# suhrig/arriba

Hardware: AMD Instinct MI355X
Metric: chimeric reads/s end-to-end (BAM->fusions.tsv), synthetic (higher is better)
Workload: dtype int32

## Files before the change

arriba_amd/csrc/device/agpu_ingest.hip:

```cpp
#include <hip/hip_runtime.h>
#include <algorithm>
#include <cstring>
#include <string>
#include <vector>
#include <rocprim/rocprim.hpp>
#include "agpu_context.hpp"
#include "ingest_core.hpp"
#include "device_utils.hpp"
#include "shard_host.hpp"
#include "crc32_core.hpp"
#include "inflate_fast_core.hpp"

using namespace agpu;
namespace agpu { extern thread_local bool g_inside_ingest_finish; }

namespace {

const int BLOCK = 256;
inline unsigned int grid_for(uint64_t n, int block = BLOCK) { return (unsigned int) ((n + block - 1) / block); }

enum { IC_ACTIVE = 0, IC_MAPPED_READS = 1, IC_MISSING_HI = 2, IC_BROKEN = 3, IC_MALFORMED = 4, IC_CHIMERIC = 5, IC_COLLISION = 6, IC_MISMATCH = 7, IC_UNSORTED = 8, IC_MAX_NAME = 9,
       IC_MAX_READ_LENGTH = 10, IC_STRAND_COUNT = 11, IC_STRAND_MATCHING = 12, IC_RUNS_UNSORTED = 13, IC_QNAME_COMMA = 14, IC_COUNT = 16 };

#define HIP_CHECK(call) do { hipError_t e_ = (call); if (e_ != hipSuccess) { set_last_error(std::string(#call) + ": " + hipGetErrorString(e_)); return AGPU_ERR_DEVICE; } } while (0)
#define ALLOC(buffer, bytes) do { if (!(buffer).allocate(bytes)) { set_last_error("hipMalloc failed (" #buffer ")"); return AGPU_ERR_NO_MEMORY; } } while (0)
#define TRY(call) do { int s_ = (call); if (s_ != AGPU_OK) return s_; } while (0)


__global__ void __launch_bounds__(BLOCK) bgzf_unwrap_kernel(const uint8_t* raw, const agpu_bgzf_block* blocks, uint8_t* stream) {
	const agpu_bgzf_block block = blocks[blockIdx.x];
	const uint8_t* source = raw + block.raw_offset + block.payload_offset;
	uint8_t* target = stream + block.stream_offset;
	const uint32_t size = block.payload_size;
	uint32_t head = (uint32_t) ((4 - ((uintptr_t) target & 3)) & 3);
	if (head > size) head = size;
	if (threadIdx.x < head) target[threadIdx.x] = source[threadIdx.x];
	const uint32_t words = (size - head) / 4;
	for (uint32_t w = threadIdx.x; w < words; w += BLOCK) *(uint32_t*) (target + head + 4 * (size_t) w) = load_u32(source + head + 4 * (size_t) w);
	const uint32_t tail = head + 4 * words;
	if (threadIdx.x < size - tail) target[tail + threadIdx.x] = source[tail + threadIdx.x];
}

template <int LANES> __global__ void __launch_bounds__(LANES) bgzf_inflate_tokens_kernel(const uint8_t* raw, const agpu_bgzf_block* blocks, uint32_t n_blocks, uint8_t* stream, uint8_t* spill,
                                                                                        unsigned long long* notes, uint32_t* note_count, int* status, unsigned int* failures) {
	__shared__ InflateFastTables tables[LANES];
	const uint32_t b = blockIdx.x * LANES + threadIdx.x;
	if (b >= n_blocks) return;
	const agpu_bgzf_block block = blocks[b];
	const bool partial = block.skip != 0 || block.keep != block.isize;
	uint8_t* target = partial ? spill + (b == 0 ? 0 : 65536) : stream + block.stream_offset;
	uint32_t noted = 0;
	const int result = block.isize > 65536 ? (int) INFLATE_OUTPUT_OVERRUN
	                 : inflate_tokens(raw + block.raw_offset + block.payload_offset, block.payload_size, target, block.isize, notes + (size_t) b * INFLATE_MATCH_CAPACITY, INFLATE_MATCH_CAPACITY, noted, tables[threadIdx.x]);
	note_count[b] = noted; status[b] = result;
	if (result != INFLATE_OK && result != INFLATE_RETRY) atomicAdd(failures, 1u);
}

__global__ void __launch_bounds__(BLOCK) bgzf_inflate_resolve_kernel(const agpu_bgzf_block* blocks, uint32_t n_blocks, uint8_t* stream, uint8_t* spill, const unsigned long long* notes, const uint32_t* note_count, const int* status) {
	const uint32_t b = blockIdx.x * (BLOCK / 64) + (threadIdx.x >> 6), lane = threadIdx.x & 63;
	if (b >= n_blocks || status[b] != INFLATE_OK) return;
	const agpu_bgzf_block block = blocks[b];
	const bool partial = block.skip != 0 || block.keep != block.isize;
	uint8_t* target = partial ? spill + (b == 0 ? 0 : 65536) : stream + block.stream_offset;
	const unsigned long long* mine = notes + (size_t) b * INFLATE_MATCH_CAPACITY;
	const uint32_t n = note_count[b];
	for (uint32_t base = 0; base < n; base += 64) {
		const unsigned long long note = base + lane < n ? mine[base + lane] : 0ull;
		const uint32_t position = inflate_note_position(note), length = inflate_note_length(note), distance = inflate_note_distance(note);
		bool pending = base + lane < n;
		while (true) {
			const unsigned long long waiting = __ballot(pending);
			if (waiting == 0) break;
			const uint32_t frontier = (uint32_t) __shfl((int) position, __ffsll((unsigned long long) waiting) - 1);
			if (pending && inflate_match_is_ready(position, length, distance, frontier)) { inflate_copy_match(target, position, length, distance); pending = false; }
			__builtin_amdgcn_fence(__ATOMIC_SEQ_CST, "workgroup");
		}
	}
	if (partial) for (uint32_t k = lane; k < block.keep; k += 64) stream[block.stream_offset + k] = target[block.skip + k];
}

__global__ void __launch_bounds__(64, 3) bgzf_inflate_kernel(const uint8_t* raw, const agpu_bgzf_block* blocks, uint8_t* stream, uint8_t* spill, int* status, int* verdict, unsigned int* failures) {
	__shared__ InflateShared shared;
	if (status != nullptr && status[blockIdx.x] != INFLATE_RETRY) return;
	const agpu_bgzf_block block = blocks[blockIdx.x];
	const bool partial = block.skip != 0 || block.keep != block.isize;
	uint8_t* target = partial ? spill + (blockIdx.x == 0 ? 0 : 65536) : stream + block.stream_offset;
	auto sync = [] () { __syncthreads(); };
	auto broadcast = [] (uint32_t value) { return (uint32_t) __builtin_amdgcn_readfirstlane((int) value); };
	const int result = inflate_block(raw + block.raw_offset + block.payload_offset, block.payload_size, target, block.isize, shared, threadIdx.x, 64u, sync, broadcast);
	if (verdict != nullptr && threadIdx.x == 0) verdict[blockIdx.x] = result;
	if (result != INFLATE_OK) { if (threadIdx.x == 0) atomicAdd(failures, 1u); return; }
	if (partial) {
		__syncthreads();
		for (uint32_t k = threadIdx.x; k < block.keep; k += 64) stream[block.stream_offset + k] = __hip_atomic_load(&target[block.skip + k], __ATOMIC_RELAXED, __HIP_MEMORY_SCOPE_AGENT);
	}
}


__global__ void segment_guess_kernel(const uint8_t* bytes, uint64_t size, uint64_t base, uint64_t segment_begin, uint64_t n_segments, uint32_t n_targets, uint64_t* first, uint64_t* end, uint32_t* count) {
	const uint64_t s = segment_begin + blockIdx.x * (uint64_t) BLOCK + threadIdx.x;
	if (s < n_segments) guess_segment(bytes, size, base, s, n_targets, first, end, count);
}

__global__ void segment_check_kernel(const uint64_t* first, const uint64_t* end, uint64_t segment_begin, uint64_t n_segments, uint8_t* mismatch, uint32_t* mismatches) {
	__shared__ uint32_t block_sum;
	uint32_t mine = 0;
	for (uint64_t s = segment_begin + blockIdx.x * (uint64_t) BLOCK + threadIdx.x; s < n_segments; s += gridDim.x * (uint64_t) BLOCK) {
		const bool bad = s > 0 && first[s] != end[s - 1];
		mismatch[s] = bad;
		mine += bad;
	}
	block_tally(mine, mismatches, &block_sum);
}

__global__ void segment_repair_kernel(const uint8_t* bytes, uint64_t size, uint64_t base, uint64_t segment_begin, uint64_t n_segments, const uint8_t* mismatch, const uint64_t* previous_end, uint64_t* first, uint64_t* end, uint32_t* count) {
	const uint64_t s = segment_begin + blockIdx.x * (uint64_t) BLOCK + threadIdx.x;
	if (s < n_segments) repair_segment_run(bytes, size, base, n_segments, s, mismatch, previous_end, first, end, count);
}

__global__ void segment_emit_kernel(const uint8_t* bytes, uint64_t size, uint64_t base, uint64_t segment_begin, uint64_t n_segments, const uint64_t* first, const uint32_t* record_base, uint64_t* record_offset) {
	const uint64_t s = segment_begin + blockIdx.x * (uint64_t) BLOCK + threadIdx.x;
	if (s >= n_segments) return;
	const uint64_t begin = base + s * SEGMENT_BYTES, segment_end = (begin + SEGMENT_BYTES < size) ? begin + SEGMENT_BYTES : size;
	uint32_t n = 0;
	walk_segment(bytes, size, first[s], segment_end, n, record_offset + record_base[s]);
}


const uint32_t PARSE_WINDOW = 16384;
__global__ void __launch_bounds__(BLOCK) record_parse_kernel(IngestStream in, GenomeView genome, uint64_t seed, uint64_t record_begin, uint64_t* keys, uint8_t* bits, int32_t* hit_index, uint32_t* counters) {
	__shared__ uint32_t sums[4];
	__shared__ __attribute__((aligned(16))) uint8_t staged[BLOCK / 64][PARSE_WINDOW + 64];
	const uint32_t wave = threadIdx.x / 64, lane = threadIdx.x % 64;
	uint8_t* window = staged[wave];
	uint32_t active = 0, mapped = 0, missing = 0, broken = 0;
	for (uint64_t base = record_begin + ((uint64_t) blockIdx.x * (BLOCK / 64) + wave) * 64; base < in.n_records; base += (uint64_t) gridDim.x * BLOCK) {
		const uint64_t r = base + lane;
		const uint64_t piece_begin = in.record_offset[base] & ~15ull, piece_end = base + 64 < in.n_records ? in.record_offset[base + 64] : in.size;
		const bool in_lds = piece_end > piece_begin && piece_end - piece_begin <= PARSE_WINDOW;
		if (in_lds) {
			for (uint64_t at = piece_begin + 16 * lane; at < piece_end; at += 16 * 64) *(uint4*) (window + (at - piece_begin)) = *(const uint4*) (in.bytes + at);
			__builtin_amdgcn_fence(__ATOMIC_RELEASE, "workgroup"); __builtin_amdgcn_wave_barrier(); __builtin_amdgcn_fence(__ATOMIC_ACQUIRE, "workgroup");
		}
		if (r < in.n_records) {
			const uint64_t offset = in.record_offset[r];
			const uint8_t* p = in.bytes + offset;
			uint32_t block_size = load_u32(p);
			if (in_lds && offset + 4 + (uint64_t) block_size <= piece_end && offset + 36 <= piece_end) { p = window + (offset - piece_begin); block_size = load_u32(p); }
			uint64_t key = ~0ull;
			uint8_t status = RECORD_SKIPPED;
			int32_t hit = HIT_INDEX_UNKNOWN;
			if (!record_sizes_ok(p + 4, block_size)) { status = RECORD_BROKEN; ++broken; }
			else {
				const Rec record = load_record_at(in, p);
				if (!((record.flag & BAMF_UNMAP) || ((record.flag & BAMF_PAIRED) && (record.flag & BAMF_MUNMAP)))) {
					const AuxTags tags = scan_aux(record.aux, record.end);
					if (!tags.has_hi && (record.flag & BAMF_SECONDARY)) { status = RECORD_MISSING_HI; ++missing; }
					else if (record.contig < 0) { status = RECORD_BROKEN; ++broken; }
					else {
						status = RECORD_ACTIVE | (tags.has_sa ? RECORD_HAS_SA : 0);
						key = name_key(record, tags.has_hi ? tags.hi : 1, seed);
						hit = hit_index_to_keep(tags);
						++active;
						if (!(record.flag & BAMF_SUPPLEMENTARY) && (genome.contig_bits[record.contig] & CBIT_INTERESTING)) ++mapped;
					}
				}
			}
			keys[r] = key;
			bits[r] = status;
			hit_index[r] = hit;
		}
		__builtin_amdgcn_fence(__ATOMIC_RELEASE, "workgroup"); __builtin_amdgcn_wave_barrier();
	}
	block_tally(active, &counters[IC_ACTIVE], &sums[0]);
	block_tally(mapped, &counters[IC_MAPPED_READS], &sums[1]);
	block_tally(missing, &counters[IC_MISSING_HI], &sums[2]);
	block_tally(broken, &counters[IC_BROKEN], &sums[3]);
}

__global__ void group_head_kernel(const uint64_t* sorted_keys, uint64_t n_active, uint8_t* head) {
	const uint64_t p = blockIdx.x * (uint64_t) BLOCK + threadIdx.x;
	if (p < n_active) head[p] = p == 0 || sorted_keys[p] != sorted_keys[p - 1];
}
__global__ void group_first_flag_kernel(const uint32_t* sorted_records, const uint32_t* group_start, uint32_t n_groups, uint8_t* first_flags) {
	const uint32_t g = blockIdx.x * BLOCK + threadIdx.x;
	if (g < n_groups) first_flags[sorted_records[group_start[g]]] = 1;
}
__global__ void group_rank_kernel(const uint32_t* sorted_records, const uint32_t* group_start, uint32_t n_groups, uint64_t n_active, const uint32_t* stream_rank, uint32_t* group_first, uint32_t* group_begin, uint32_t* group_count) {
	const uint32_t g = blockIdx.x * BLOCK + threadIdx.x;
	if (g >= n_groups) return;
	const uint32_t begin = group_start[g], first = sorted_records[begin], t = stream_rank[first];
	group_first[t] = first; group_begin[t] = begin; group_count[t] = (uint32_t) ((g + 1 < n_groups ? (uint64_t) group_start[g + 1] : n_active) - begin);
}
__global__ void group_names_kernel(IngestStream in, const uint32_t* sorted_records, const uint32_t* group_begin, const uint32_t* group_count, uint32_t first_group, uint32_t n_groups, uint32_t* counters) {
	const uint32_t t = first_group + blockIdx.x * BLOCK + threadIdx.x;
	if (t >= n_groups || group_count[t] < 2) return;
	const uint32_t* records = sorted_records + group_begin[t];
	const Rec a = load_record(in, records[0]);
	const int64_t hit_a = hit_index_of(in, records[0], a);
	for (uint32_t k = 1; k < group_count[t]; ++k) {
		const Rec b = load_record(in, records[k]);
		if (!same_name(a, hit_a, b, hit_index_of(in, records[k], b))) { atomicOr(&counters[IC_COLLISION], 1u); return; }
	}
}


__global__ void window_carry_kernel(uint32_t* record_base, uint64_t segment_begin, uint64_t segment_end, const uint32_t* records_before) {
	const uint64_t s = segment_begin + blockIdx.x * (uint64_t) BLOCK + threadIdx.x;
	if (s <= segment_end) record_base[s] += *records_before;
}
__global__ void window_summary_kernel(const uint32_t* record_base, const uint64_t* end, uint64_t segment_end, uint32_t* records_before, uint32_t* words) {
	*records_before = record_base[segment_end];
	words[1] = record_base[segment_end];
	const uint64_t last_end = end[segment_end - 1];
	words[4] = (uint32_t) last_end; words[5] = (uint32_t) (last_end >> 32);
}
struct RecordIsActive { __host__ __device__ bool operator()(uint8_t bits) const { return (bits & RECORD_STATUS_MASK) == RECORD_ACTIVE; } };
__global__ void run_head_kernel(const uint64_t* keys, const uint32_t* active_records, uint64_t begin, uint64_t end, uint8_t* head) {
	const uint64_t i = begin + blockIdx.x * (uint64_t) BLOCK + threadIdx.x;
	if (i < end) head[i] = i == 0 || keys[active_records[i]] != keys[active_records[i - 1]];
}
__global__ void run_close_kernel(const uint32_t* active_records, const uint32_t* run_begin, uint32_t first_group, uint32_t n_groups, uint32_t n_runs, uint64_t active_total, uint32_t* group_first, uint32_t* group_count) {
	const uint32_t g = first_group + blockIdx.x * BLOCK + threadIdx.x;
	if (g >= n_groups) return;
	const uint32_t begin = run_begin[g];
	group_first[g] = active_records[begin];
	group_count[g] = (uint32_t) ((g + 1 < n_runs ? (uint64_t) run_begin[g + 1] : active_total) - begin);
}
__global__ void run_key_kernel(const uint64_t* keys, const uint32_t* group_first, uint32_t n_groups, uint64_t* out) {
	const uint32_t g = blockIdx.x * BLOCK + threadIdx.x;
	if (g < n_groups) out[g] = keys[group_first[g]];
}
__global__ void run_repeat_kernel(const uint64_t* sorted_keys, uint32_t n_groups, uint32_t* repeats) {
	__shared__ uint32_t block_sum;
	uint32_t mine = 0;
	for (uint64_t g = blockIdx.x * (uint64_t) BLOCK + threadIdx.x; g < n_groups; g += gridDim.x * (uint64_t) BLOCK) mine += g > 0 && sorted_keys[g] == sorted_keys[g - 1];
	block_tally(mine, repeats, &block_sum);
}

struct ViralCounter {
	unsigned long long* counts;
	__device__ void operator()(uint32_t contig) { atomicAdd(&counts[contig], 1ull); }
};

#ifndef AGPU_REPLAY_WAVES
#define AGPU_REPLAY_WAVES 0
#endif
#ifndef AGPU_PACK_WAVES
#define AGPU_PACK_WAVES 0
#endif
#if AGPU_REPLAY_WAVES > 0
#define AGPU_REPLAY_OCCUPANCY __attribute__((amdgpu_waves_per_eu(AGPU_REPLAY_WAVES, AGPU_REPLAY_WAVES)))
#else
#define AGPU_REPLAY_OCCUPANCY
#endif
#if AGPU_PACK_WAVES > 0
#define AGPU_PACK_OCCUPANCY __attribute__((amdgpu_waves_per_eu(AGPU_PACK_WAVES, AGPU_PACK_WAVES)))
#else
#define AGPU_PACK_OCCUPANCY
#endif
template <bool RUNS> __global__ void __launch_bounds__(BLOCK) AGPU_REPLAY_OCCUPANCY group_replay_kernel(IngestContext ctx, const uint32_t* sorted_records, const uint32_t* group_begin, const uint32_t* group_count, uint32_t first_group, uint32_t n_groups,
                                                             FragmentPlan* plain, TandemPlan* itd, uint8_t* valid, FragmentSizes* sizes, unsigned long long* viral_counts, uint32_t* qname_differs, uint32_t* counters) {
	__shared__ uint32_t sums[2];
	GroupTally tally; tally.malformed = 0; tally.chimeric = 0; tally.collision = 0;
	const uint32_t g = first_group + blockIdx.x * BLOCK + threadIdx.x;
	if (g < n_groups) {
		const uint32_t begin = group_begin[g];
		const uint32_t n_records = group_count[g];
		const Rec representative = load_record(ctx.stream, sorted_records[begin]);
		const int64_t hit = hit_index_of(ctx.stream, sorted_records[begin], representative);
		const uint32_t length = qname_length(representative);
		if (RUNS) {
			if (find_byte(representative.name, length, ',') < length) atomicOr(&counters[IC_QNAME_COMMA], 1u);
			if (g == 0) qname_differs[0] = 0;
			else {
				const uint32_t record_before = sorted_records[group_begin[g - 1]];
				const Rec run_before = load_record(ctx.stream, record_before);
				const uint32_t length_before = qname_length(run_before), shorter = length < length_before ? length : length_before, different = first_difference(run_before.name, representative.name, shorter);
				qname_differs[g] = length != length_before || different < shorter;
				bool unsorted;
				if (different < shorter) unsorted = run_before.name[different] > representative.name[different];
				else unsorted = compare_names(fragment_name(run_before, hit_index_of(ctx.stream, record_before, run_before), false, length_before), fragment_name(representative, hit, false, length)) >= 0;
				if (unsorted) atomicOr(&counters[IC_RUNS_UNSORTED], 1u);
			}
		}
		FragmentPlan plain_plan; TandemPlan itd_plan;
		ViralCounter viral = { viral_counts };
		replay_group(ctx, sorted_records + begin, n_records, plain_plan, itd_plan, tally, viral, RUNS ? &representative : nullptr, length, hit);
		if (tally.collision) atomicOr(&counters[IC_COLLISION], 1u);
		Fragment3 fragment;
		AGPU_NOUNROLL for (uint32_t entry = 0; entry < 2; ++entry) {
			const FragmentPlan& plan = entry ? itd_plan.plan : plain_plan;
			bool ok = false;
			if (plan.count > 0) {
				ok = normalize_plan(ctx.stream, plan, entry ? &itd_plan.tandem : nullptr, fragment);
				if (!ok) tally.malformed++;
			}
			valid[2 * (size_t) g + entry] = ok;
			FragmentSizes mine; mine.cigar_words = 0; mine.sequence_bytes = 0; mine.name_length = 0;
			if (ok) { if (entry) itd[g] = itd_plan; else plain[g] = plain_plan; fragment_sizes(fragment, representative, hit, entry, mine, length); }
			sizes[2 * (size_t) g + entry] = mine;
		}
	}
	block_tally(tally.malformed, &counters[IC_MALFORMED], &sums[0]);
	block_tally(tally.chimeric, &counters[IC_CHIMERIC], &sums[1]);
}


__device__ FragmentName name_of(const IngestStream& in, const uint32_t* group_first, uint32_t ref, Rec& storage) {
	storage = load_record(in, group_first[ref >> 1]);
	return fragment_name(storage, hit_index_of(in, group_first[ref >> 1], storage), ref & 1);
}

__global__ void name_order_check_kernel(IngestStream in, const uint32_t* group_first, const uint32_t* order, uint64_t n, uint32_t* counters) {
	__shared__ uint32_t block_max;
	if (threadIdx.x == 0) block_max = 0;
	__syncthreads();
	const uint64_t i = blockIdx.x * (uint64_t) BLOCK + threadIdx.x;
	if (i < n) {
		Rec storage_a, storage_b;
		const FragmentName mine = name_of(in, group_first, order[i], storage_a);
		atomicMax(&block_max, name_length(mine));
		if (i > 0) {
			const FragmentName before = name_of(in, group_first, order[i - 1], storage_b);
			if (compare_names(before, mine) >= 0) atomicOr(&counters[IC_UNSORTED], 1u);
		}
	}
	__syncthreads();
	if (threadIdx.x == 0 && block_max) atomicMax(&counters[IC_MAX_NAME], block_max);
}

__global__ void run_itd_order_kernel(IngestStream in, const uint32_t* group_first, const uint8_t* valid, uint32_t first_group, uint32_t n_groups, uint32_t* counters) {
	const uint32_t g = first_group + blockIdx.x * BLOCK + threadIdx.x;
	if (g >= n_groups || g == 0 || !valid[2 * (size_t) (g - 1) + 1]) return;
	Rec storage_a, storage_b;
	const FragmentName mine = name_of(in, group_first, 2 * g, storage_b);
	const FragmentName before = name_of(in, group_first, 2 * (g - 1) + 1, storage_a);
	if (compare_names(before, mine) >= 0) atomicOr(&counters[IC_RUNS_UNSORTED], 1u);
}

__global__ void name_chunk_kernel(IngestStream in, const uint32_t* group_first, const uint32_t* order, uint64_t n, uint32_t chunk, uint64_t* keys) {
	const uint64_t i = blockIdx.x * (uint64_t) BLOCK + threadIdx.x;
	if (i >= n) return;
	Rec storage;
	keys[i] = name_chunk(name_of(in, group_first, order[i], storage), chunk);
}


__global__ void fragment_layout_kernel(IngestStream in, const uint32_t* group_first, const uint32_t* order, uint64_t n, const FragmentSizes* sizes, const uint32_t* qname_run ,
                                       uint32_t* cigar_words, uint32_t* sequence_bytes, uint32_t* name_lengths, uint32_t* new_group) {
	const uint64_t i = blockIdx.x * (uint64_t) BLOCK + threadIdx.x;
	if (i > n) return;
	if (i == n) { cigar_words[i] = 0; sequence_bytes[i] = 0; name_lengths[i] = 0; return; }
	const uint32_t ref = order[i];
	const FragmentSizes mine = sizes[ref];
	cigar_words[i] = mine.cigar_words; sequence_bytes[i] = mine.sequence_bytes; name_lengths[i] = mine.name_length;
	uint32_t differs = 0;
	if (i > 0 && qname_run != nullptr) differs = qname_run[ref >> 1] != qname_run[order[i - 1] >> 1];
	else if (i > 0) {
		const Rec a = load_record(in, group_first[ref >> 1]), b = load_record(in, group_first[order[i - 1] >> 1]);
		const uint32_t length = qname_length(a);
		differs = length != qname_length(b);
		for (uint32_t k = 0; k < length && !differs; ++k) differs = a.name[k] != b.name[k];
	}
	new_group[i] = differs;
}

__global__ void __launch_bounds__(BLOCK) AGPU_PACK_OCCUPANCY fragment_pack_kernel(IngestStream in, const uint32_t* group_first, const uint32_t* order, uint64_t n, const FragmentPlan* plain, const TandemPlan* itd,
                                                              const uint64_t* cigar_base, const uint64_t* sequence_base, const uint64_t* name_base, const uint32_t* group_id, PackTarget out, uint32_t* counters) {
	__shared__ uint32_t block_max;
	if (threadIdx.x == 0) block_max = 0;
	__syncthreads();
	const uint64_t i = blockIdx.x * (uint64_t) BLOCK + threadIdx.x;
	if (i == n) out.name_offset[n] = name_base[n];
	if (i < n) {
		const uint32_t ref = order[i], g = ref >> 1;
		const bool is_itd = ref & 1;
		Fragment3 f;
		normalize_plan(in, is_itd ? itd[g].plan : plain[g], is_itd ? &itd[g].tandem : nullptr, f);
		Rec storage;
		const FragmentName name = name_of(in, group_first, ref, storage);
		atomicMax(&block_max, write_fragment(in, f, name, i, cigar_base[i], sequence_base[i], name_base[i], group_id[i], out));
	}
	__syncthreads();
	if (threadIdx.x == 0 && block_max) atomicMax(&counters[IC_MAX_READ_LENGTH], block_max);
}

template <bool INFLATED> __global__ void __launch_bounds__(256) bgzf_crc_kernel(const uint8_t* raw, const agpu_bgzf_block* blocks, uint32_t n_blocks, const Crc32Tables* tables, unsigned int* mismatches) {
	__shared__ uint32_t slice[4][256];
	__shared__ uint32_t join[2][4][256];
	__shared__ uint32_t staged[4][CRC32_WAVE_LANES * (CRC32_ROUND_WORDS + 1)];
	for (uint32_t k = threadIdx.x; k < 4 * 256; k += 256) ((uint32_t*) slice)[k] = ((const uint32_t*) tables->slice)[k];
	for (uint32_t k = threadIdx.x; k < 2 * 4 * 256; k += 256) ((uint32_t*) join)[k] = ((const uint32_t*) tables->join)[k];
	const uint32_t wave = threadIdx.x / CRC32_WAVE_LANES, lane = threadIdx.x % CRC32_WAVE_LANES, b = blockIdx.x * 4 + wave;
	agpu_bgzf_block block;
	block.crc32 = 0; block.payload_size = 0; block.raw_offset = 0; block.payload_offset = 0;
	if (b < n_blocks) block = blocks[b];
	if (INFLATED) { block.raw_offset = block.stream_offset; block.payload_offset = 0; block.payload_size = block.isize; }
	const bool checked = b < n_blocks && block.crc32 != 0 && block.payload_size <= CRC32_VIRTUAL;
	const uint8_t* payload = raw + block.raw_offset + block.payload_offset;
	const uint32_t n = block.payload_size;
	uint32_t* mine = staged[wave];
	uint32_t c = 0;
	const bool by_chunks = checked && n >= 4;
	const uint32_t first_word = by_chunks ? (CRC32_VIRTUAL - n) / 4 : CRC32_VIRTUAL / 4;
	for (uint32_t round = 0; round < CRC32_WAVE_CHUNK / 4 / CRC32_ROUND_WORDS; ++round) {
		__syncthreads();
		for (uint32_t item = lane; item < CRC32_WAVE_LANES * CRC32_ROUND_WORDS; item += CRC32_WAVE_LANES) {
			const uint32_t chunk = item / CRC32_ROUND_WORDS, j = item % CRC32_ROUND_WORDS, w = chunk * (CRC32_WAVE_CHUNK / 4) + round * CRC32_ROUND_WORDS + j;
			mine[chunk * (CRC32_ROUND_WORDS + 1) + j] = w >= first_word ? crc32_virtual_word(payload, n, w) : 0u;
		}
		__syncthreads();
		for (uint32_t j = 0; j < CRC32_ROUND_WORDS; ++j) c = crc32_raw_step(slice, c, mine[lane * (CRC32_ROUND_WORDS + 1) + j]);
	}
	__syncthreads();
	mine[lane] = c;
	__syncthreads();
	if (lane % 8 == 0) { for (uint32_t i = 1; i < 8; ++i) c = crc32_apply(join[0], c) ^ mine[lane + i]; }
	__syncthreads();
	if (lane % 8 == 0) mine[lane] = c;
	__syncthreads();
	if (lane == 0 && checked) {
		for (uint32_t g = 1; g < 8; ++g) c = crc32_apply(join[1], c) ^ mine[8 * g];
		c ^= 0xFFFFFFFFu;
		if (n < 4) c = crc32_of_sliced(slice, payload, n);
		if (c != block.crc32) atomicAdd(mismatches, 1u);
	}
}

__global__ void shard_rebase_kernel(uint32_t* out, const uint32_t* in, uint64_t n, uint32_t base, const uint8_t* n_aln, uint32_t slot) {
	const uint64_t i = (uint64_t) blockIdx.x * blockDim.x + threadIdx.x;
	if (i < n) out[i] = in[i] + ((slot >= 3 || slot < n_aln[i]) ? base : 0u);
}
__global__ void shard_rebase_names_kernel(uint64_t* out, const uint64_t* in, uint64_t n, uint64_t base) {
	const uint64_t i = (uint64_t) blockIdx.x * blockDim.x + threadIdx.x;
	if (i < n) out[i] = in[i] + base;
}
__global__ void shard_add_coverage_kernel(uint32_t* windows, uint8_t* starts, uint8_t* ends, const uint32_t* part_windows, const uint8_t* part_starts, const uint8_t* part_ends, uint64_t n) {
	const uint64_t i = (uint64_t) blockIdx.x * blockDim.x + threadIdx.x;
	if (i < n) { windows[i] += part_windows[i]; starts[i] |= part_starts[i]; ends[i] |= part_ends[i]; }
}
__global__ void shard_add_counts_kernel(unsigned long long* counts, const unsigned long long* part, uint32_t n) {
	const uint32_t i = blockIdx.x * blockDim.x + threadIdx.x;
	if (i < n) counts[i] += part[i];
}

__global__ void packed_name_length_kernel(const uint64_t* name_offset, uint64_t n, uint32_t* longest) {
	const uint64_t i = blockIdx.x * (uint64_t) BLOCK + threadIdx.x;
	if (i < n) atomicMax(longest, (uint32_t) (name_offset[i + 1] - name_offset[i]));
}
__global__ void packed_name_chunk_kernel(const char* names, const uint64_t* name_offset, const uint32_t* order, uint64_t n, uint32_t chunk, uint64_t* keys) {
	const uint64_t i = blockIdx.x * (uint64_t) BLOCK + threadIdx.x;
	if (i >= n) return;
	const uint32_t row = order[i]; const uint64_t begin = name_offset[row]; const uint32_t length = (uint32_t) (name_offset[row + 1] - begin);
	uint64_t key = 0;
	for (uint32_t k = 0; k < 8; ++k) { const uint32_t at = 8 * chunk + k; key = key << 8 | (at < length ? (uint8_t) names[begin + at] : 0u); }
	keys[i] = key;
}
__global__ void packed_name_neighbours_kernel(const char* names, const uint64_t* name_offset, const uint32_t* order, uint64_t n, uint32_t* new_group, uint32_t* equal_names) {
	const uint64_t i = blockIdx.x * (uint64_t) BLOCK + threadIdx.x;
	if (i >= n) return;
	if (i == 0) { new_group[0] = 0; return; }
	const uint32_t a = order[i - 1], b = order[i]; const uint64_t begin_a = name_offset[a], begin_b = name_offset[b]; const uint32_t length_a = (uint32_t) (name_offset[a + 1] - begin_a), length_b = (uint32_t) (name_offset[b + 1] - begin_b);
	bool same = length_a == length_b;
	for (uint32_t k = 0; same && k < length_a; ++k) same = names[begin_a + k] == names[begin_b + k];
	if (same) atomicAdd(equal_names, 1u);
	uint32_t qname_a = length_a, qname_b = length_b;
	while (qname_a > 0 && names[begin_a + qname_a - 1] != ',') --qname_a;
	while (qname_b > 0 && names[begin_b + qname_b - 1] != ',') --qname_b;
	bool same_qname = qname_a == qname_b;
	for (uint32_t k = 0; same_qname && k < qname_a; ++k) same_qname = names[begin_a + k] == names[begin_b + k];
	new_group[i] = same_qname ? 0u : 1u;
}
__global__ void qname_run_flag_kernel(IngestStream in, uint64_t n_records, uint8_t* flags) {
	const uint64_t r = blockIdx.x * (uint64_t) BLOCK + threadIdx.x;
	if (r < n_records) flags[r] = starts_qname_run(in, (uint32_t) r) ? 1 : 0;
}
__global__ void qname_key_kernel(IngestStream in, const uint32_t* run_starts, uint64_t n_runs, uint64_t* keys) {
	const uint64_t k = blockIdx.x * (uint64_t) BLOCK + threadIdx.x;
	if (k < n_runs) qname_key128(load_record(in, run_starts[k]), keys[2 * k], keys[2 * k + 1]);
}
__global__ void qname_low_kernel(const uint64_t* keys, uint64_t n, uint64_t* low) { const uint64_t k = blockIdx.x * (uint64_t) BLOCK + threadIdx.x; if (k < n) low[k] = keys[2 * k]; }
__global__ void qname_equal_kernel(const uint64_t* low_sorted, const uint32_t* index_sorted, const uint64_t* keys, uint64_t n, uint32_t* equal) {
	const uint64_t k = blockIdx.x * (uint64_t) BLOCK + threadIdx.x;
	if (k > 0 && k < n && low_sorted[k] == low_sorted[k - 1] && keys[2 * (uint64_t) index_sorted[k] + 1] == keys[2 * (uint64_t) index_sorted[k - 1] + 1]) atomicAdd(equal, 1u);
}
__global__ void iota_kernel(uint32_t* out, uint64_t n) { const uint64_t i = blockIdx.x * (uint64_t) BLOCK + threadIdx.x; if (i < n) out[i] = (uint32_t) i; }

__global__ void coverage_from_differences_kernel(const uint32_t* summed, const uint64_t* window_offset, uint32_t n_contigs, uint64_t n, uint32_t* counts, uint16_t* out) {
	const uint64_t i = blockIdx.x * (uint64_t) BLOCK + threadIdx.x;
	if (i >= n) return;
	uint32_t low = 0, high = n_contigs;
	while (high - low > 1) { const uint32_t middle = (low + high) / 2; if (window_offset[middle] <= i) low = middle; else high = middle; }
	const uint32_t count = summed[i + low];
	counts[i] = count;
	out[i] = count > 65535u ? (uint16_t) 65535 : (uint16_t) count;
}
__global__ void coverage_clamp_kernel(const uint32_t* windows, uint64_t n, uint16_t* out) {
	const uint64_t i = blockIdx.x * (uint64_t) BLOCK + threadIdx.x;
	if (i < n) out[i] = windows[i] > 65535u ? (uint16_t) 65535 : (uint16_t) windows[i];
}


__global__ void gather_sizes_kernel(BatchView b, const uint64_t* name_offset, const uint32_t* ids, uint64_t n, uint32_t* cigar_words, uint32_t* sequence_bytes, uint32_t* name_lengths) {
	const uint64_t k = blockIdx.x * (uint64_t) BLOCK + threadIdx.x;
	if (k > n) return;
	if (k == n) { cigar_words[k] = 0; sequence_bytes[k] = 0; name_lengths[k] = 0; return; }
	row_sizes(b, name_offset, ids ? ids[k] : k, cigar_words[k], sequence_bytes[k], name_lengths[k]);
}

__global__ void gather_copy_kernel(BatchView b, const uint8_t* pristine_fbits, const uint8_t* const* pristine_abits, const uint64_t* name_offset, const char* names, const uint32_t* ids, uint64_t n,
                                   const uint64_t* cigar_base, const uint64_t* sequence_base, const uint64_t* name_base, PackTarget out) {
	const uint64_t k = blockIdx.x * (uint64_t) BLOCK + threadIdx.x;
	if (k == n) { if (out.name_offset) out.name_offset[n] = name_base[n]; else out.row_name_offset[n] = (uint32_t) name_base[n]; }
	if (k >= n) return;
	copy_row(b, pristine_fbits, pristine_abits, name_offset, names, ids ? ids[k] : k, k, cigar_base[k], sequence_base[k], name_base[k], out);
}


__global__ void strandedness_flag_kernel(BatchView b, AnnotationView ann, uint64_t first, uint64_t count, uint8_t* flags) {
	const uint64_t k = blockIdx.x * (uint64_t) BLOCK + threadIdx.x;
	if (k >= count) return;
	flags[k] = strandedness_vote(b, ann, first + k);
}

__global__ void strandedness_take_kernel(const uint8_t* flags, uint64_t count, uint32_t wanted, uint32_t* counters) {
	if (blockIdx.x != 0 || threadIdx.x != 0) return;
	uint32_t seen = counters[IC_STRAND_COUNT], matching = counters[IC_STRAND_MATCHING];
	for (uint64_t k = 0; k < count && seen < wanted; ++k)
		if (flags[k]) { ++seen; if (flags[k] & 2) ++matching; }
	counters[IC_STRAND_COUNT] = seen; counters[IC_STRAND_MATCHING] = matching;
}


int grow_stream(agpu_ctx* ctx, uint64_t needed) {
	needed += 64;
	if (needed <= ctx->ingest_stream.capacity) { ctx->ingest_stream.bytes = needed; return AGPU_OK; }
	DeviceBuffer larger;
	const uint64_t doubled = ctx->ingest_stream.capacity * 2;
	if (!larger.allocate(std::max<uint64_t>(needed + (needed >> 3), std::max<uint64_t>(doubled, 64u << 20)))) { set_last_error("hipMalloc failed (BAM stream)"); return AGPU_ERR_NO_MEMORY; }
	if (ctx->piece_stream) { HIP_CHECK(hipStreamSynchronize(ctx->piece_stream)); HIP_CHECK(hipStreamSynchronize(ctx->piece_stream2)); }
	if (ctx->ingest_stream_size > 0) HIP_CHECK(hipMemcpyAsync(larger.ptr, ctx->ingest_stream.ptr, ctx->ingest_stream_size, hipMemcpyDeviceToDevice, ctx->stream));
	HIP_CHECK(hipStreamSynchronize(ctx->stream));
	if (ctx->ingest_progress.work) HIP_CHECK(hipStreamSynchronize(ctx->ingest_progress.work));
	ctx->ingest_stream.swap(larger);
	return AGPU_OK;
}

int wait_for_previous_push(agpu_ctx* ctx) {
	const uint32_t behind = ctx->ingest_host_buffers - 1;
	if (ctx->ingest_pushes >= behind) HIP_CHECK(hipEventSynchronize(ctx->piece_copied[(ctx->ingest_pushes - behind) % AGPU_PIECE_SLOTS]));
	return AGPU_OK;
}

template <class Key> int sort_pairs(agpu_ctx* ctx, DeviceBuffer& scratch, Key* keys_in, Key* keys_out, uint32_t* values_in, uint32_t* values_out, uint64_t n, unsigned int end_bit, const char* label, bool counting_values) {
	size_t bytes = 0;
	hipStream_t s = ctx->stream;
	if (counting_values) HIP_CHECK(rocprim::radix_sort_pairs(nullptr, bytes, keys_in, keys_out, rocprim::counting_iterator<uint32_t>(0), values_out, n, 0, end_bit, s));
	else HIP_CHECK(rocprim::radix_sort_pairs(nullptr, bytes, keys_in, keys_out, values_in, values_out, n, 0, end_bit, s));
	if (bytes > scratch.capacity) ALLOC(scratch, bytes);
	KernelTimer timer(ctx, label, n * (uint64_t) (sizeof(Key) + 4) * 2);
	if (counting_values) HIP_CHECK(rocprim::radix_sort_pairs(scratch.ptr, bytes, keys_in, keys_out, rocprim::counting_iterator<uint32_t>(0), values_out, n, 0, end_bit, s));
	else HIP_CHECK(rocprim::radix_sort_pairs(scratch.ptr, bytes, keys_in, keys_out, values_in, values_out, n, 0, end_bit, s));
	return AGPU_OK;
}

int select_flagged(agpu_ctx* ctx, DeviceBuffer& scratch, const uint8_t* flags, uint32_t* out, uint32_t* device_count, uint64_t n) {
	size_t bytes = 0;
	HIP_CHECK(rocprim::select(nullptr, bytes, rocprim::counting_iterator<uint32_t>(0), flags, out, device_count, n, ctx->stream));
	if (bytes > scratch.capacity) ALLOC(scratch, bytes);
	HIP_CHECK(rocprim::select(scratch.ptr, bytes, rocprim::counting_iterator<uint32_t>(0), flags, out, device_count, n, ctx->stream));
	return AGPU_OK;
}

int exclusive_sum_u64(agpu_ctx* ctx, DeviceBuffer& scratch, const uint32_t* in, uint64_t* out, uint64_t n) {
	size_t bytes = 0;
	HIP_CHECK(rocprim::exclusive_scan(nullptr, bytes, in, out, (uint64_t) 0, n, rocprim::plus<uint64_t>(), ctx->stream));
	if (bytes > scratch.capacity) ALLOC(scratch, bytes);
	HIP_CHECK(rocprim::exclusive_scan(scratch.ptr, bytes, in, out, (uint64_t) 0, n, rocprim::plus<uint64_t>(), ctx->stream));
	return AGPU_OK;
}


const unsigned int INGEST_WINDOW_RING = 16, INGEST_WINDOW_WORDS = 8;
uint64_t g_window_bytes = 512u << 20;
uint64_t g_window_margin = 1u << 20;

int grow_keeping(agpu_ctx* ctx, DeviceBuffer& buffer, size_t needed, size_t used, size_t estimate) {
	if (needed == 0) needed = 16;
	if (buffer.ptr != nullptr && needed <= buffer.capacity) { if (needed > buffer.bytes) buffer.bytes = needed; return AGPU_OK; }
	DeviceBuffer larger;
	if (!larger.allocate(std::max(needed + needed / 2, estimate)) && !larger.allocate(needed)) { set_last_error("hipMalloc failed (tables of the ingest)"); return AGPU_ERR_NO_MEMORY; }
	hipStream_t s = ctx->ingest_progress.work;
	if (used > 0 && buffer.ptr != nullptr) HIP_CHECK(hipMemcpyAsync(larger.ptr, buffer.ptr, std::min(used, buffer.capacity), hipMemcpyDeviceToDevice, s));
	HIP_CHECK(hipStreamSynchronize(s));
	buffer.swap(larger);
	return AGPU_OK;
}

IngestStream window_stream(agpu_ctx* ctx, uint64_t size, uint64_t n_records) {
	IngestStream in;
	in.bytes = ctx->ingest_stream.as<uint8_t>(); in.size = size; in.record_offset = ctx->scratch("ingest.record_offset").as<uint64_t>(); in.n_records = n_records;
	in.n_targets = ctx->ingest_n_targets; in.tid_to_contig = ctx->ingest_tid_to_contig.as<uint32_t>();
	in.hit_index = ctx->scratch("ingest.hit_index").as<int32_t>();
	return in;
}

IngestContext replay_context(agpu_ctx* ctx, const IngestStream& in) {
	IngestContext context;
	context.stream = in; context.annotation = ctx->annotation; context.annotation.n_dummy = 0; context.genome = ctx->genome;
	context.coverage.n_contigs = ctx->genome.n_contigs; context.coverage.window_offset = ctx->coverage_window_offset.as<uint64_t>(); context.coverage.windows = ctx->coverage_windows32.as<uint32_t>();
	context.coverage.fragment_starts = ctx->coverage_fragment_starts.as<uint8_t>(); context.coverage.fragment_ends = ctx->coverage_fragment_ends.as<uint8_t>();
	if (getenv("ARRIBA_INGEST_SKIP_COVERAGE") != nullptr) context.coverage.windows = nullptr;
	context.record_bits = ctx->scratch("ingest.record_bits").as<uint8_t>(); context.max_itd_length = ctx->ingest_max_itd_length; context.external_duplicate_marking = ctx->ingest_external_duplicate_marking;
	return context;
}

int window_step(agpu_ctx* ctx, IngestWindow& w) {
	IngestProgress& p = ctx->ingest_progress;
	hipStream_t s = p.work;
	uint32_t* words = ctx->scratch("ingest.window_words").as<uint32_t>() + (size_t) w.slot * INGEST_WINDOW_WORDS;
	uint32_t* device_counters = ctx->scratch("ingest.counters").as<uint32_t>();
	DeviceBuffer& rocprim_scratch = ctx->scratch("ingest.window_rocprim");
	const uint64_t base = ctx->ingest_first_record;
	const uint8_t* bytes = ctx->ingest_stream.as<uint8_t>();
	const uint64_t n = w.segment_end - w.segment_begin;
	const size_t estimated_records = (size_t) (p.size_hint / 128 + 4096);
	size_t temporary = 0;
	switch (w.enqueued + 1) {
	case 1: {
		HIP_CHECK(hipMemsetAsync(words, 0, INGEST_WINDOW_WORDS * 4, s));
		if (n == 0) break;
		DeviceBuffer& first = ctx->scratch("ingest.segment_first"); DeviceBuffer& end = ctx->scratch("ingest.segment_end"); DeviceBuffer& end_before = ctx->scratch("ingest.segment_end_before");
		DeviceBuffer& count = ctx->scratch("ingest.segment_count"); DeviceBuffer& record_base = ctx->scratch("ingest.segment_base"); DeviceBuffer& mismatch = ctx->scratch("ingest.segment_mismatch");
		const size_t segments = (size_t) w.segment_end + 1, done = (size_t) w.segment_begin + 1, estimate = (size_t) (p.size_hint / SEGMENT_BYTES + 16);
		TRY(grow_keeping(ctx, first, segments * 8, done * 8, estimate * 8)); TRY(grow_keeping(ctx, end, segments * 8, done * 8, estimate * 8)); TRY(grow_keeping(ctx, end_before, segments * 8, 0, estimate * 8));
		TRY(grow_keeping(ctx, count, segments * 4, done * 4, estimate * 4)); TRY(grow_keeping(ctx, record_base, segments * 4, done * 4, estimate * 4)); TRY(grow_keeping(ctx, mismatch, segments, done, estimate));
		{ KernelTimer timer(ctx, "segment_guess_kernel", n * SEGMENT_BYTES, s);
		  segment_guess_kernel<<<grid_for(n), BLOCK, 0, s>>>(bytes, w.avail, base, w.segment_begin, w.segment_end, ctx->ingest_n_targets, first.as<uint64_t>(), end.as<uint64_t>(), count.as<uint32_t>()); }
		for (int pass = 0; pass < 3; ++pass) {
			segment_check_kernel<<<tally_grid(n, BLOCK), BLOCK, 0, s>>>(first.as<uint64_t>(), end.as<uint64_t>(), w.segment_begin, w.segment_end, mismatch.as<uint8_t>(), words + 6);
			const uint64_t from = w.segment_begin > 0 ? w.segment_begin - 1 : 0;
			HIP_CHECK(hipMemcpyAsync(end_before.as<uint64_t>() + from, end.as<uint64_t>() + from, (w.segment_end - from) * 8, hipMemcpyDeviceToDevice, s));
			segment_repair_kernel<<<grid_for(n), BLOCK, 0, s>>>(bytes, w.avail, base, w.segment_begin, w.segment_end, mismatch.as<uint8_t>(), end_before.as<uint64_t>(), first.as<uint64_t>(), end.as<uint64_t>(), count.as<uint32_t>());
		}
		segment_check_kernel<<<tally_grid(n, BLOCK), BLOCK, 0, s>>>(first.as<uint64_t>(), end.as<uint64_t>(), w.segment_begin, w.segment_end, mismatch.as<uint8_t>(), words + 0);
		HIP_CHECK(hipMemsetAsync(count.as<uint32_t>() + w.segment_end, 0, 4, s));
		HIP_CHECK(rocprim::exclusive_scan(nullptr, temporary, count.as<uint32_t>() + w.segment_begin, record_base.as<uint32_t>() + w.segment_begin, 0u, n + 1, rocprim::plus<uint32_t>(), s));
		if (temporary > rocprim_scratch.capacity) ALLOC(rocprim_scratch, temporary);
		HIP_CHECK(rocprim::exclusive_scan(rocprim_scratch.ptr, temporary, count.as<uint32_t>() + w.segment_begin, record_base.as<uint32_t>() + w.segment_begin, 0u, n + 1, rocprim::plus<uint32_t>(), s));
		uint32_t* records_before = ctx->scratch("ingest.window_state").as<uint32_t>();
		window_carry_kernel<<<grid_for(n + 1), BLOCK, 0, s>>>(record_base.as<uint32_t>(), w.segment_begin, w.segment_end, records_before);
		window_summary_kernel<<<1, 1, 0, s>>>(record_base.as<uint32_t>(), end.as<uint64_t>(), w.segment_end, records_before, words);
		break; }
	case 2: {
		const uint64_t records = w.record_end - w.record_begin;
		w.active_begin = p.active;
		if (records == 0) break;
		DeviceBuffer& record_offset = ctx->scratch("ingest.record_offset"); DeviceBuffer& keys = ctx->scratch("ingest.keys"); DeviceBuffer& record_bits = ctx->scratch("ingest.record_bits"); DeviceBuffer& active_records = ctx->scratch("ingest.sorted_records");
		TRY(grow_keeping(ctx, record_offset, w.record_end * 8, w.record_begin * 8, estimated_records * 8)); TRY(grow_keeping(ctx, keys, w.record_end * 8, w.record_begin * 8, estimated_records * 8));
		TRY(grow_keeping(ctx, ctx->scratch("ingest.hit_index"), w.record_end * 4, w.record_begin * 4, estimated_records * 4));
		TRY(grow_keeping(ctx, record_bits, w.record_end, w.record_begin, estimated_records)); TRY(grow_keeping(ctx, active_records, (w.active_begin + records) * 4, w.active_begin * 4, estimated_records * 4));
		{ KernelTimer timer(ctx, "segment_emit_kernel", records * 8, s);
		  segment_emit_kernel<<<grid_for(n), BLOCK, 0, s>>>(bytes, w.avail, base, w.segment_begin, w.segment_end, ctx->scratch("ingest.segment_first").as<uint64_t>(), ctx->scratch("ingest.segment_base").as<uint32_t>(), record_offset.as<uint64_t>()); }
		const IngestStream in = window_stream(ctx, w.avail, w.record_end);
		{ KernelTimer timer(ctx, "record_parse_kernel", records * (8 + 64 + 9), s);
		  record_parse_kernel<<<tally_grid(records, BLOCK) * 8, BLOCK, 0, s>>>(in, ctx->genome, 0, w.record_begin, keys.as<uint64_t>(), record_bits.as<uint8_t>(), ctx->scratch("ingest.hit_index").as<int32_t>(), device_counters); }
		auto flags = rocprim::make_transform_iterator(record_bits.as<uint8_t>() + w.record_begin, RecordIsActive());
		HIP_CHECK(rocprim::select(nullptr, temporary, rocprim::counting_iterator<uint32_t>((uint32_t) w.record_begin), flags, active_records.as<uint32_t>() + w.active_begin, words + 2, records, s));
		if (temporary > rocprim_scratch.capacity) ALLOC(rocprim_scratch, temporary);
		HIP_CHECK(rocprim::select(rocprim_scratch.ptr, temporary, rocprim::counting_iterator<uint32_t>((uint32_t) w.record_begin), flags, active_records.as<uint32_t>() + w.active_begin, words + 2, records, s));
		break; }
	case 3: {
		const uint64_t active = w.active_end - w.active_begin;
		w.head_begin = p.heads;
		if (active == 0) break;
		DeviceBuffer& head = ctx->scratch("ingest.head"); DeviceBuffer& run_begin = ctx->scratch("ingest.group_begin");
		TRY(grow_keeping(ctx, head, w.active_end, 0, estimated_records)); TRY(grow_keeping(ctx, run_begin, (w.head_begin + active + 1) * 4, w.head_begin * 4, estimated_records * 2));
		{ KernelTimer timer(ctx, "run_head_kernel", active * (8 + 4 + 1), s);
		  run_head_kernel<<<grid_for(active), BLOCK, 0, s>>>(ctx->scratch("ingest.keys").as<uint64_t>(), ctx->scratch("ingest.sorted_records").as<uint32_t>(), w.active_begin, w.active_end, head.as<uint8_t>()); }
		HIP_CHECK(rocprim::select(nullptr, temporary, rocprim::counting_iterator<uint32_t>((uint32_t) w.active_begin), head.as<uint8_t>() + w.active_begin, run_begin.as<uint32_t>() + w.head_begin, words + 3, active, s));
		if (temporary > rocprim_scratch.capacity) ALLOC(rocprim_scratch, temporary);
		HIP_CHECK(rocprim::select(rocprim_scratch.ptr, temporary, rocprim::counting_iterator<uint32_t>((uint32_t) w.active_begin), head.as<uint8_t>() + w.active_begin, run_begin.as<uint32_t>() + w.head_begin, words + 3, active, s));
		break; }
	case 4: {
// ... 1161 lines not shown
```

arriba_amd/csrc/device/ingest_core.hpp:

```cpp
#ifndef AGPU_INGEST_CORE_HPP
#define AGPU_INGEST_CORE_HPP 1

#include "annotate_core.hpp"
#include "event_core.hpp"

namespace agpu {


AGPU_HD uint32_t load_u32(const uint8_t* p) { uint32_t v; __builtin_memcpy(&v, p, 4); return v; }
AGPU_HD uint64_t load_u64(const uint8_t* p) { uint64_t v; __builtin_memcpy(&v, p, 8); return v; }
AGPU_HD uint32_t first_zero_byte(uint64_t v) { const uint64_t z = (v - 0x0101010101010101ull) & ~v & 0x8080808080808080ull; return z ? (uint32_t) __builtin_ctzll(z) >> 3 : 8u; }
AGPU_HD uint64_t low_bytes(uint32_t n) { return n >= 8 ? ~0ull : (1ull << (8 * n)) - 1; }
AGPU_HD uint32_t find_byte(const uint8_t* p, uint32_t n, uint8_t byte) {
	const uint64_t pattern = 0x0101010101010101ull * byte;
	uint32_t i = 0;
	for (; i + 8 <= n; i += 8) { const uint32_t z = first_zero_byte(load_u64(p + i) ^ pattern); if (z < 8) return i + z; }
	if (i == n) return n;
	if (n >= 8) {
		const uint32_t z = first_zero_byte((load_u64(p + n - 8) ^ pattern) | low_bytes(i - (n - 8)));
		return z < 8 ? n - 8 + z : n;
	}
	for (; i < n; ++i) if (p[i] == byte) return i;
	return n;
}
AGPU_HD uint32_t first_difference(const uint8_t* a, const uint8_t* b, uint32_t n) {
	uint32_t i = 0;
	for (; i + 8 <= n; i += 8) { const uint64_t x = load_u64(a + i) ^ load_u64(b + i); if (x) return i + ((uint32_t) __builtin_ctzll(x) >> 3); }
	if (i == n) return n;
	if (n >= 8) {
		const uint64_t x = (load_u64(a + n - 8) ^ load_u64(b + n - 8)) & ~low_bytes(i - (n - 8));
		return x ? n - 8 + ((uint32_t) __builtin_ctzll(x) >> 3) : n;
	}
	for (; i < n; ++i) if (a[i] != b[i]) return i;
	return n;
}
AGPU_HD uint16_t load_u16(const uint8_t* p) { uint16_t v; __builtin_memcpy(&v, p, 2); return v; }

enum : uint16_t { BAMF_PAIRED = 1, BAMF_PROPER_PAIR = 2, BAMF_UNMAP = 4, BAMF_MUNMAP = 8, BAMF_REVERSE = 16, BAMF_READ1 = 64, BAMF_SECONDARY = 256, BAMF_DUP = 1024, BAMF_SUPPLEMENTARY = 2048 };

AGPU_HD bool op_consumes_query(uint32_t op) { return (0x3C1A7u >> (op << 1)) & 1; }
AGPU_HD bool op_consumes_reference(uint32_t op) { return (0x3C1A7u >> (op << 1)) & 2; }

struct IngestStream {
	const uint8_t* bytes;
	uint64_t size;
	const uint64_t* record_offset;
	uint64_t n_records;
	uint32_t n_targets;
	const uint32_t* tid_to_contig;
	const int32_t* hit_index;
};
const int32_t HIT_INDEX_UNKNOWN = -0x7FFFFFFF - 1;

struct Rec {
	const uint8_t* cigar_bytes; const uint8_t* seq_bytes; const uint8_t* name; const uint8_t* aux; const uint8_t* end;
	int32_t contig, pos, l_seq;
	uint32_t n_cigar, l_read_name;
	uint16_t flag;
	AGPU_HD uint32_t cigar(uint32_t i) const { return load_u32(cigar_bytes + 4 * (size_t) i); }
	AGPU_HD uint32_t op(uint32_t i) const { return cigar(i) & 15; }
	AGPU_HD uint32_t len(uint32_t i) const { return cigar(i) >> 4; }
	AGPU_HD uint32_t code(int32_t i) const { return (seq_bytes[i >> 1] >> ((~i & 1) << 2)) & 15; }
	AGPU_HD bool forward() const { return !(flag & BAMF_REVERSE); }
	AGPU_HD bool paired() const { return flag & BAMF_PAIRED; }
	AGPU_HD int32_t qlen(uint32_t n) const { int32_t l = 0; for (uint32_t i = 0; i < n; ++i) if (op_consumes_query(op(i))) l += (int32_t) len(i); return l; }
	AGPU_HD int32_t rlen(uint32_t n) const { int32_t l = 0; for (uint32_t i = 0; i < n; ++i) if (op_consumes_reference(op(i))) l += (int32_t) len(i); return l; }
	AGPU_HD int32_t endpos() const { int32_t l = (!(flag & BAMF_UNMAP) && n_cigar > 0) ? rlen(n_cigar) : 1; return pos + (l == 0 ? 1 : l); }
};

AGPU_HD bool record_sizes_ok(const uint8_t* block, uint32_t block_size) {
	if (block_size < 32) return false;
	const uint32_t l_read_name = block[8], n_cigar = load_u16(block + 12);
	const int32_t l_seq = (int32_t) load_u32(block + 16);
	if (l_seq < 0 || l_read_name == 0) return false;
	const uint64_t fixed = 32ull + l_read_name + 4ull * n_cigar + ((uint64_t) l_seq + 1) / 2 + (uint64_t) l_seq;
	return fixed <= block_size;
}

AGPU_HD Rec load_record_at(const IngestStream& in, const uint8_t* p) {
	const uint64_t word0 = load_u64(p), word1 = load_u64(p + 8), word2 = load_u64(p + 16);
	const uint32_t block_size = (uint32_t) word0;
	p += 4;
	Rec rec;
	const int32_t tid = (int32_t) (word0 >> 32);
	rec.contig = (tid >= 0 && (uint32_t) tid < in.n_targets) ? (int32_t) in.tid_to_contig[tid] : -1;
	rec.pos = (int32_t) (uint32_t) word1;
	rec.l_read_name = (uint32_t) (word1 >> 32) & 0xFFu;
	rec.n_cigar = (uint32_t) word2 & 0xFFFFu;
	rec.flag = (uint16_t) (word2 >> 16);
	rec.l_seq = (int32_t) (word2 >> 32);
	rec.name = p + 32;
	rec.cigar_bytes = rec.name + rec.l_read_name;
	rec.seq_bytes = rec.cigar_bytes + 4 * (size_t) rec.n_cigar;
	rec.aux = rec.seq_bytes + ((size_t) rec.l_seq + 1) / 2 + (size_t) rec.l_seq;
	rec.end = p + block_size;
	return rec;
}
AGPU_HD Rec load_record(const IngestStream& in, uint32_t r) { return load_record_at(in, in.bytes + in.record_offset[r]); }


const uint32_t SEGMENT_BYTES = 8192;
const uint64_t SEARCH_LIMIT = 4u << 20;
const uint64_t OFFSET_NONE = ~0ull, OFFSET_BROKEN = ~0ull - 1;

AGPU_HD bool plausible_record(const uint8_t* bytes, uint64_t size, uint64_t o, uint32_t n_targets) {
	if (o + 36 > size) return false;
	const uint32_t block_size = load_u32(bytes + o);
	if (block_size < 32 || block_size > (1u << 28) || o + 4 + (uint64_t) block_size > size) return false;
	const uint8_t* p = bytes + o + 4;
	const int32_t tid = (int32_t) load_u32(p), pos = (int32_t) load_u32(p + 4), next_tid = (int32_t) load_u32(p + 20), next_pos = (int32_t) load_u32(p + 24);
	if (tid < -1 || tid >= (int32_t) n_targets || next_tid < -1 || next_tid >= (int32_t) n_targets || pos < -1 || next_pos < -1) return false;
	if (!record_sizes_ok(p, block_size)) return false;
	const uint32_t l_read_name = p[8];
	return p[32 + l_read_name - 1] == 0;
}

AGPU_HD uint64_t walk_segment(const uint8_t* bytes, uint64_t size, uint64_t start, uint64_t segment_end, uint32_t& count, uint64_t* offsets) {
	uint64_t o = start;
	count = 0;
	while (o < segment_end) {
		if (o + 4 > size) return OFFSET_BROKEN;
		const uint32_t block_size = load_u32(bytes + o);
		if (block_size < 32 || o + 4 + (uint64_t) block_size > size) return OFFSET_BROKEN;
		if (offsets != nullptr) offsets[count] = o;
		++count;
		o += 4 + (uint64_t) block_size;
	}
	return o;
}

AGPU_HD void guess_segment(const uint8_t* bytes, uint64_t size, uint64_t base, uint64_t s, uint32_t n_targets, uint64_t* first, uint64_t* end, uint32_t* count) {
	const uint64_t begin = base + s * SEGMENT_BYTES, segment_end = (begin + SEGMENT_BYTES < size) ? begin + SEGMENT_BYTES : size;
	uint64_t start = OFFSET_NONE;
	if (s == 0) start = base;
	else {
		const uint64_t limit = (begin + SEARCH_LIMIT < size) ? begin + SEARCH_LIMIT : size;
		for (uint64_t o = begin; o < limit; ++o) {
			if (!plausible_record(bytes, size, o, n_targets)) continue;
			const uint64_t next = o + 4 + (uint64_t) load_u32(bytes + o);
			if (next == size || plausible_record(bytes, size, next, n_targets)) { start = o; break; }
		}
	}
	first[s] = start;
	uint32_t n = 0;
	end[s] = (start == OFFSET_NONE) ? OFFSET_NONE : walk_segment(bytes, size, start, segment_end, n, nullptr);
	count[s] = n;
}

AGPU_HD void repair_segment_run(const uint8_t* bytes, uint64_t size, uint64_t base, uint64_t n_segments, uint64_t s, const uint8_t* mismatch, const uint64_t* previous_end, uint64_t* first, uint64_t* end, uint32_t* count) {
	if (!mismatch[s] || mismatch[s - 1]) return;
	uint64_t start = previous_end[s - 1];
	for (uint64_t t = s; t < n_segments && (t == s || mismatch[t]); ++t) {
		const uint64_t begin = base + t * SEGMENT_BYTES, segment_end = (begin + SEGMENT_BYTES < size) ? begin + SEGMENT_BYTES : size;
		first[t] = start;
		uint32_t n = 0;
		end[t] = (start >= OFFSET_BROKEN) ? start : walk_segment(bytes, size, start, segment_end, n, nullptr);
		count[t] = n;
		start = end[t];
	}
}

struct AuxTags { bool has_hi, has_sa; int64_t hi; };
AGPU_HD AuxTags scan_aux(const uint8_t* s, const uint8_t* end) {
	AuxTags tags; tags.has_hi = false; tags.has_sa = false; tags.hi = 0;
	while (s + 3 <= end) {
		const uint8_t* value = s + 2;
		size_t size;
		switch (*value) {
			case 'A': case 'c': case 'C': size = 2; break;
			case 's': case 'S': size = 3; break;
			case 'i': case 'I': case 'f': size = 5; break;
			case 'd': size = 9; break;
			case 'Z': case 'H': { const uint8_t* p = value + 1; while (p < end && *p) ++p; if (p >= end) return tags; size = (size_t) (p - value) + 1; break; }
			case 'B': {
				if (value + 6 > end) return tags;
				const size_t element = (value[1] == 'c' || value[1] == 'C') ? 1 : (value[1] == 's' || value[1] == 'S') ? 2 : 4;
				size = 6 + element * (size_t) load_u32(value + 2);
				break;
			}
			default: return tags;
		}
		if (value + size > end) return tags;
		if (s[0] == 'H' && s[1] == 'I' && !tags.has_hi) {
			tags.has_hi = true;
			switch (*value) {
				case 'c': tags.hi = (int8_t) value[1]; break;
				case 'C': tags.hi = value[1]; break;
				case 's': tags.hi = (int16_t) load_u16(value + 1); break;
				case 'S': tags.hi = load_u16(value + 1); break;
				case 'i': tags.hi = (int32_t) load_u32(value + 1); break;
				case 'I': tags.hi = load_u32(value + 1); break;
				default: tags.hi = 0; break;
			}
		}
		if (s[0] == 'S' && s[1] == 'A') tags.has_sa = true;
		if (tags.has_hi && tags.has_sa) return tags;
		s = value + size;
	}
	return tags;
}

AGPU_HD int32_t hit_index_to_keep(const AuxTags& tags) { const int64_t hi = tags.has_hi ? tags.hi : 1; return (hi > HIT_INDEX_UNKNOWN && hi <= 0x7FFFFFFF) ? (int32_t) hi : HIT_INDEX_UNKNOWN; }
AGPU_HD int64_t hit_index_of(const IngestStream& in, uint32_t record, const Rec& rec) {
	if (in.hit_index != nullptr) { const int32_t kept = in.hit_index[record]; if (kept != HIT_INDEX_UNKNOWN) return kept; }
	const AuxTags tags = scan_aux(rec.aux, rec.end);
	return tags.has_hi ? tags.hi : 1;
}

enum : uint8_t { RECORD_SKIPPED = 0, RECORD_ACTIVE = 1, RECORD_MISSING_HI = 2, RECORD_BROKEN = 3, RECORD_STATUS_MASK = 3, RECORD_HAS_SA = 4 };

AGPU_HD uint32_t qname_length(const Rec& r) { return find_byte(r.name, r.l_read_name, 0); }

AGPU_HD bool starts_qname_run(const IngestStream& in, uint32_t record) {
	if (record == 0) return true;
	const Rec a = load_record(in, record - 1), b = load_record(in, record);
	const uint32_t length = qname_length(b);
	if (qname_length(a) != length) return true;
	for (uint32_t i = 0; i < length; ++i) if (a.name[i] != b.name[i]) return true;
	return false;
}
AGPU_HD void qname_key128(const Rec& r, uint64_t& low, uint64_t& high) {
	uint64_t h = 1469598103934665603ull, g = 0x9AE16A3B2F90404Full;
	for (uint32_t i = 0; i < r.l_read_name && r.name[i]; ++i) { h = (h ^ r.name[i]) * 1099511628211ull; g = (g ^ (r.name[i] + 0x9Eu)) * 0x100000001B3ull; g ^= g >> 29; }
	h ^= h >> 33; h *= 0xFF51AFD7ED558CCDull; h ^= h >> 33; h *= 0xC4CEB9FE1A85EC53ull; h ^= h >> 33;
	g ^= g >> 31; g *= 0x7FB5D329728EA185ull; g ^= g >> 27; g *= 0x81DADEF4BC2DD44Dull; g ^= g >> 33;
	low = h; high = g;
}

AGPU_HD uint64_t name_key(const Rec& r, int64_t hit_index, uint64_t seed) {
	uint64_t h = 1469598103934665603ull ^ seed;
	for (uint32_t i = 0; i < r.l_read_name && r.name[i]; ++i) h = (h ^ r.name[i]) * 1099511628211ull;
	h ^= (uint64_t) hit_index * 0x9E3779B97F4A7C15ull;
	h ^= h >> 33; h *= 0xFF51AFD7ED558CCDull; h ^= h >> 33; h *= 0xC4CEB9FE1A85EC53ull; h ^= h >> 33;
	return h == ~0ull ? ~0ull - 1 : h;
}
AGPU_HD bool same_name(const Rec& a, uint32_t length_a , int64_t hi_a, const Rec& b, int64_t hi_b) {
	if (hi_a != hi_b) return false;
	if (length_a != qname_length(b)) return false;
	return first_difference(a.name, b.name, length_a) == length_a;
}
AGPU_HD bool same_name(const Rec& a, int64_t hi_a, const Rec& b, int64_t hi_b) { return same_name(a, qname_length(a), hi_a, b, hi_b); }


enum : uint8_t { CLIP_NONE = 0, CLIP_START = 1, CLIP_END = 2, PLAN_TANDEM = 3 };
const uint32_t NO_RECORD = 0xFFFFFFFFu;

struct PlanEntry { uint32_t record; uint16_t cigar_index; uint8_t clip; uint8_t supplementary; };
struct TandemAlignment { int32_t start, end; uint32_t cigar[3]; uint32_t record; uint8_t n_cigar, strand, first_in_pair, supplementary; };
struct FragmentPlan {
	PlanEntry entry[3];
	uint8_t count;
	uint8_t single_end, duplicate, reserved;
};
struct TandemPlan { FragmentPlan plan; TandemAlignment tandem; };

AGPU_HD void plan_clear(FragmentPlan& plan) { plan.count = 0; plan.single_end = 0; plan.duplicate = 0; plan.reserved = 0; for (int k = 0; k < 3; ++k) { plan.entry[k].record = NO_RECORD; plan.entry[k].cigar_index = 0; plan.entry[k].clip = 0; plan.entry[k].supplementary = 0; } }
AGPU_HD void plan_push(FragmentPlan& plan, uint32_t record, const Rec& r, bool is_supplementary, uint32_t cigar_index, uint8_t clip) {
	plan.single_end = !(r.flag & BAMF_PAIRED);
	plan.duplicate = plan.duplicate || (r.flag & BAMF_DUP);
	if (plan.count < 3) {
		PlanEntry& e = plan.entry[plan.count];
		e.record = record; e.cigar_index = (uint16_t) cigar_index; e.clip = clip; e.supplementary = is_supplementary;
	}
	if (plan.count < 255) ++plan.count;
}
AGPU_HD void plan_push_tandem(FragmentPlan& plan) {
	if (plan.count < 3) { PlanEntry& e = plan.entry[plan.count]; e.record = NO_RECORD; e.cigar_index = 0; e.clip = PLAN_TANDEM; e.supplementary = 0; }
	if (plan.count < 255) ++plan.count;
}

struct Aln {
	const uint8_t* cigar_bytes;
	uint32_t record;
	uint32_t sequence_record;
	int32_t sequence_length;
	int32_t contig, start, end;
	uint32_t n_cigar;
	uint32_t cigar_index;
	uint32_t patch_index[2], patch_value[2];
	uint32_t tandem_cigar[3];
	uint32_t made_index, made_value, shift;
	uint8_t clip, n_patch;
	bool supplementary, first_in_pair, strand;
	AGPU_HD uint32_t base_cigar(uint32_t i) const {
		if (clip == PLAN_TANDEM) return i == 0 ? tandem_cigar[0] : i == 1 ? tandem_cigar[1] : tandem_cigar[2];
		if (i == made_index) return made_value;
		return load_u32(cigar_bytes + 4 * (size_t) (i + shift));
	}
	AGPU_HD uint32_t cigar(uint32_t i) const {
		uint32_t value = base_cigar(i);
		for (uint32_t k = 0; k < n_patch; ++k) if (patch_index[k] == i) value = patch_value[k];
		return value;
	}
	AGPU_HD void set_cigar(uint32_t i, uint32_t value) {
		for (uint32_t k = 0; k < n_patch; ++k) if (patch_index[k] == i) { patch_value[k] = value; return; }
		if (n_patch < 2) { patch_index[n_patch] = i; patch_value[n_patch] = value; ++n_patch; }
	}
	AGPU_HD uint32_t preclipping() const { const uint32_t c = cigar(0), op = c & 15; return (op == CIGAR_S || op == CIGAR_H) ? c >> 4 : 0; }
	AGPU_HD uint32_t postclipping() const { const uint32_t c = cigar(n_cigar - 1), op = c & 15; return (op == CIGAR_S || op == CIGAR_H) ? c >> 4 : 0; }
};

AGPU_HD Aln materialize(const IngestStream& in, const PlanEntry& e, const TandemAlignment* tandem) {
	Aln a;
	a.n_patch = 0; a.patch_index[0] = a.patch_index[1] = 0; a.patch_value[0] = a.patch_value[1] = 0;
	a.tandem_cigar[0] = a.tandem_cigar[1] = a.tandem_cigar[2] = 0;
	a.clip = e.clip; a.cigar_index = e.cigar_index;
	a.made_index = NO_RECORD; a.made_value = 0; a.shift = 0;
	if (e.clip == PLAN_TANDEM) {
		const Rec source = load_record(in, tandem->record);
		a.cigar_bytes = source.cigar_bytes;
		a.record = NO_RECORD;
		a.supplementary = tandem->supplementary; a.first_in_pair = tandem->first_in_pair; a.strand = tandem->strand;
		a.contig = source.contig; a.start = tandem->start; a.end = tandem->end;
		a.n_cigar = tandem->n_cigar;
		for (int k = 0; k < 3; ++k) a.tandem_cigar[k] = tandem->cigar[k];
		a.sequence_record = a.supplementary ? NO_RECORD : tandem->record;
		a.sequence_length = a.supplementary ? 0 : source.l_seq;
		return a;
	}
	const Rec r = load_record(in, e.record);
	a.cigar_bytes = r.cigar_bytes;
	a.record = e.record;
	a.strand = r.forward(); a.first_in_pair = r.flag & BAMF_READ1; a.contig = r.contig; a.supplementary = e.supplementary;
	a.sequence_record = e.supplementary ? NO_RECORD : e.record;
	a.sequence_length = e.supplementary ? 0 : r.l_seq;
	if (e.clip == CLIP_START) {
		a.start = r.pos + r.rlen(e.cigar_index); a.end = r.endpos() - 1;
		a.n_cigar = r.n_cigar - e.cigar_index + 1;
		a.made_index = 0; a.made_value = (uint32_t) r.qlen(e.cigar_index) << 4 | (r.op(0) == CIGAR_H ? CIGAR_H : CIGAR_S);
		a.shift = (uint32_t) e.cigar_index - 1u;
	} else if (e.clip == CLIP_END) {
		a.start = r.pos; a.end = r.pos + r.rlen((uint32_t) e.cigar_index + 1) - 1;
		a.n_cigar = (uint32_t) e.cigar_index + 2;
		a.made_index = (uint32_t) e.cigar_index + 1; a.made_value = (uint32_t) (r.l_seq - r.qlen((uint32_t) e.cigar_index + 1)) << 4 | (r.op(r.n_cigar - 1) == CIGAR_H ? CIGAR_H : CIGAR_S);
	} else {
		a.start = r.pos; a.end = r.endpos() - 1;
		a.n_cigar = r.n_cigar;
	}
	return a;
}


AGPU_HD bool is_clipped_at_correct_end(const Rec& r) {
	if (!(r.flag & BAMF_PAIRED)) return true;
	if (r.n_cigar == 0) return false;
	uint32_t clipped_end;
	if (r.flag & BAMF_SUPPLEMENTARY) clipped_end = r.forward() ? r.n_cigar - 1 : 0;
	else clipped_end = r.forward() ? 0 : r.n_cigar - 1;
	const uint32_t op = r.op(clipped_end);
	return op == CIGAR_S || op == CIGAR_H;
}

AGPU_HD bool is_pristine_alignment(const Rec& r) {
	for (uint32_t i = 0; i < r.n_cigar; ++i) {
		const uint32_t op = r.op(i);
		if (op != CIGAR_N && op != CIGAR_M && op != CIGAR_X) return false;
	}
	const uint32_t size = (uint32_t) r.l_seq;
	for (uint32_t i = 2, repeat = 0, count = 1; i + 2 < size; i += 2) {
		if (r.code(i) == r.code(repeat) && r.code(i + 1) == r.code(repeat + 1)) {
			count++;
		} else if (r.code(i + 1) == r.code(repeat + 1) && r.code(i + 2) == r.code(repeat + 2)) {
			count++;
			i++;
		} else {
			count = 1;
			repeat = i;
		}
		if (count >= 8) return false;
	}
	return true;
}

AGPU_HD bool clipped_sequence_is_adapter(const Rec& mate1, const Rec* mate2) {
	if (mate2 == nullptr) return false;
	if (mate1.pos == mate2->pos && mate1.n_cigar > 0 && mate2->n_cigar > 0) {
		if (!mate1.forward() && mate1.op(0) == CIGAR_S && mate2->forward() && mate2->op(mate2->n_cigar - 1) == CIGAR_S && mate1.len(0) == mate2->len(mate2->n_cigar - 1)) return true;
		if (!mate2->forward() && mate2->op(0) == CIGAR_S && mate1.forward() && mate1.op(mate1.n_cigar - 1) == CIGAR_S && mate2->len(0) == mate1.len(mate1.n_cigar - 1)) return true;
	}
	return false;
}

AGPU_HD char base_character(uint32_t code) {
	const uint64_t low = 0x565352474D43413Dull , high = 0x4E42444B48595754ull ;
	return (char) (((code & 8) ? high : low) >> (8 * (code & 7)));
}
AGPU_HD uint32_t nonzero_bytes(uint64_t x) {
	const uint64_t high = (x | ((x & 0x7F7F7F7F7F7F7F7Full) + 0x7F7F7F7F7F7F7F7Full)) & 0x8080808080808080ull;
	return (uint32_t) (((high >> 7) * 0x0102040810204080ull) >> 56);
}

AGPU_HD bool is_tandem_duplication(const Rec* r, uint32_t record, const GenomeView& genome, const uint32_t max_itd_length, TandemAlignment& tandem) {
	const unsigned int min_clipped_length = 12, min_duplication_length = 9, max_duplication_length = max_itd_length;
	const unsigned int max_mismatches = 1, max_non_template_bases = 6, min_alignment_length = 15;
	if (r == nullptr || r->n_cigar == 0) return false;
	unsigned int clipped_length = 0, clipped_position = 0;
	bool clipped_start = true;
	int direction = +1, window_start = 0, window_end = 0, extended_read_start = 0;
	if (r->op(0) == CIGAR_S && r->len(0) >= min_clipped_length) {
		clipped_length = r->len(0);
		clipped_position = 0;
		direction = -1;
		window_start = r->pos + min_duplication_length - clipped_length;
		window_end = r->pos + max_duplication_length - clipped_length;
		extended_read_start = r->pos - clipped_length;
		clipped_start = true;
	}
	if (r->op(r->n_cigar - 1) == CIGAR_S && r->len(r->n_cigar - 1) >= (min_clipped_length > clipped_length ? min_clipped_length : clipped_length)) {
		clipped_length = r->len(r->n_cigar - 1);
		clipped_position = r->l_seq - clipped_length;
		direction = +1;
		window_start = r->endpos() - max_duplication_length;
		window_end = r->endpos() - min_duplication_length;
		extended_read_start = r->endpos();
		clipped_start = false;
	}
	if (clipped_length == 0) return false;
	if (r->contig < 0 || (uint32_t) r->contig >= genome.n_contigs) return false;
	const uint64_t contig_begin = genome.contig_offset[r->contig];
	const uint64_t contig_size = genome.contig_offset[r->contig + 1] - contig_begin;
	if (contig_size == 0) return false;
	const char* contig_sequence = genome.bases + contig_begin;
	if ((uint64_t) (unsigned int) (window_end + max_duplication_length + clipped_length + 1) >= contig_size ||
	    window_start <= (int) (max_duplication_length + clipped_length + 1))
		return false;

	const float min_extended_align_fraction = 0.7;
	unsigned int extended_matches = 0;
	for (unsigned int read_pos = 0; read_pos < clipped_length; ++read_pos)
		if ((uint64_t) (unsigned int) (extended_read_start + read_pos) < contig_size)
			if (contig_sequence[(unsigned int) (extended_read_start + read_pos)] == base_character(r->code((int32_t) (clipped_position + read_pos))))
				extended_matches++;
	if (1.0 * extended_matches / clipped_length >= min_extended_align_fraction) return false;

	const unsigned int held = clipped_length < 16 ? clipped_length : 16;
	uint64_t read_low = 0, read_high = 0;
	for (unsigned int i = 0; i < held; ++i) {
		const int read_pos = (direction == +1) ? (int) i : (int) (clipped_length - 1 - i);
		const uint64_t character = (uint8_t) base_character(r->code((int32_t) clipped_position + read_pos));
		if (i < 8) read_low |= character << (8 * i); else read_high |= character << (8 * (i - 8));
	}
	const uint32_t held_bits = (1u << held) - 1;
	for (int contig_pos = window_start; contig_pos <= window_end; ++contig_pos) {
		if (max_mismatches == 1 && max_non_template_bases == 6) {
			uint64_t contig_low, contig_high;
			if (direction == +1) { contig_low = load_u64((const uint8_t*) contig_sequence + contig_pos); contig_high = load_u64((const uint8_t*) contig_sequence + contig_pos + 8); }
			else {
				const uint8_t* last = (const uint8_t*) contig_sequence + contig_pos + (int) clipped_length - 1;
				contig_low = __builtin_bswap64(load_u64(last - 7)); contig_high = __builtin_bswap64(load_u64(last - 15));
			}
			const uint32_t differs = (nonzero_bytes(contig_low ^ read_low) | nonzero_bytes(contig_high ^ read_high) << 8) & held_bits;
			const uint32_t counted = differs & ~0x3Fu, second = counted & (counted - 1);
			if (second != 0) {
				const uint32_t at = (uint32_t) __builtin_ctz(second);
				if ((uint32_t) __builtin_popcount(~differs & ((1u << at) - 1)) + 2 != clipped_length) continue;
			}
		}
		unsigned int matches = 0, mismatches = 0;
		int tandem_start = (int) contig_size, tandem_end = -1;
		for (unsigned int i = 0; i < clipped_length; i++) {
			const int read_pos = (direction == +1) ? (int) i : (int) (clipped_length - 1 - i);
			if (contig_sequence[contig_pos + read_pos] == base_character(r->code((int32_t) clipped_position + read_pos))) {
				matches++;
				if (contig_pos + read_pos < tandem_start) tandem_start = contig_pos + read_pos;
				if (contig_pos + read_pos > tandem_end) tandem_end = contig_pos + read_pos;
			} else if (i >= max_non_template_bases) {
				mismatches++;
				if (mismatches > max_mismatches) break;
			}
		}
		if (matches >= min_alignment_length || matches + mismatches == clipped_length) {
			tandem.start = tandem_start; tandem.end = tandem_end;
			tandem.record = record;
			tandem.strand = r->forward();
			tandem.first_in_pair = (r->flag & BAMF_READ1) != 0;
			tandem.supplementary = !(r->flag & BAMF_PAIRED) || (clipped_start && r->forward()) || (!clipped_start && !r->forward());
			uint32_t clip_left = clipped_start ? 0 : r->l_seq - clipped_length;
			uint32_t clip_right = clipped_start ? r->l_seq - clipped_length : 0;
			if (tandem_start > contig_pos) clip_left += tandem_start - contig_pos;
			if (tandem_end < contig_pos + (int) clipped_length - 1) clip_right += contig_pos + clipped_length - 1 - tandem_end;
			tandem.n_cigar = 0;
			tandem.cigar[0] = tandem.cigar[1] = tandem.cigar[2] = 0;
			if (clip_left > 0) tandem.cigar[tandem.n_cigar++] = clip_left << 4 | CIGAR_S;
			tandem.cigar[tandem.n_cigar++] = (uint32_t) (tandem_end - tandem_start + 1) << 4 | CIGAR_M;
			if (clip_right > 0) tandem.cigar[tandem.n_cigar++] = clip_right << 4 | CIGAR_S;
			return true;
		}
	}
	return false;
}

AGPU_HD bool find_spanning_intron(const Rec& r, int32_t gene1_end, int32_t gene2_start, uint32_t& cigar_index, int32_t& read_pos) {
	if (r.n_cigar < 3) return false;
	int32_t before = r.pos, after;
	for (uint32_t i = 0; i < r.n_cigar; ++i) {
		const uint32_t op = r.op(i);
		const uint32_t op_length = op_consumes_reference(op) ? r.len(i) : 0;
		after = before + (int32_t) op_length;
		if (op == CIGAR_N && ((before <= gene1_end && after > gene1_end) || (before < gene2_start && after >= gene2_start))) {
			cigar_index = i;
			read_pos = r.qlen(i);
			return true;
		}
		before = after;
	}
	return false;
}

AGPU_HD ListRef genes_at(const FlatIndexView& gene_index, int32_t contig, int32_t position) {
	if (contig < 0 || (uint32_t) contig >= gene_index.n_contigs) return empty_list();
	const uint32_t k = index_lower_bound(gene_index, (uint32_t) contig, position);
	if (k == gene_index.contig_offset[contig + 1]) return empty_list();
	return index_bucket(gene_index, k);
}
AGPU_HD bool lists_intersect(ListRef a, ListRef b) {
	uint32_t i = 0, j = 0;
	while (i < a.n && j < b.n) { const uint32_t x = a.p[i], y = b.p[j]; if (x < y) ++i; else if (y < x) ++j; else return true; }
	return false;
}
AGPU_HD void boundaries_of_biggest_gene(const AnnotationView& ann, ListRef genes, int32_t& start, int32_t& end) {
	start = -1; end = -1;
	for (uint32_t g = 0; g < genes.n; ++g) {
		const int32_t gene_start = ann.gene_start[genes.p[g]], gene_end = ann.gene_end[genes.p[g]];
		if (start == -1 || start > gene_start) start = gene_start;
		if (end == -1 || end < gene_end) end = gene_end;
	}
}

AGPU_HD bool extract_read_through_alignment(FragmentPlan& plan, uint32_t record_index, const Rec& record, uint32_t previous_index, const Rec* previous, const AnnotationView& ann) {
	const Rec* forward_mate = &record; const Rec* reverse_mate = previous;
	uint32_t forward_index = record_index, reverse_index = previous_index;
	if (!forward_mate->forward()) { const Rec* t = forward_mate; forward_mate = reverse_mate; reverse_mate = t; const uint32_t ti = forward_index; forward_index = reverse_index; reverse_index = ti; }
	ListRef forward_genes, reverse_genes;
	if (forward_mate != nullptr) forward_genes = genes_at(ann.gene_index, forward_mate->contig, forward_mate->pos);
	else forward_genes = genes_at(ann.gene_index, reverse_mate->contig, reverse_mate->pos);
	if (reverse_mate != nullptr) reverse_genes = genes_at(ann.gene_index, reverse_mate->contig, reverse_mate->endpos());
	else reverse_genes = genes_at(ann.gene_index, forward_mate->contig, forward_mate->endpos());
	const bool common_empty = !lists_intersect(forward_genes, reverse_genes);
	if (!(common_empty && !(forward_genes.n == 0 && reverse_genes.n == 0))) return false;

	int32_t forward_gene_start, forward_gene_end, reverse_gene_start, reverse_gene_end;
	boundaries_of_biggest_gene(ann, forward_genes, forward_gene_start, forward_gene_end);
	boundaries_of_biggest_gene(ann, reverse_genes, reverse_gene_start, reverse_gene_end);
	if (forward_gene_end == -1) forward_gene_end = reverse_gene_start - 1;
	if (reverse_gene_start == -1) reverse_gene_start = forward_gene_end + 1;

	uint32_t forward_cigar_op = 0, reverse_cigar_op = 0;
	int32_t forward_read_pos = 0, reverse_read_pos = 0;
	const bool forward_has_intron = (forward_mate == nullptr) ? false : find_spanning_intron(*forward_mate, forward_gene_end, reverse_gene_start, forward_cigar_op, forward_read_pos);
	const bool reverse_has_intron = (reverse_mate == nullptr) ? false : find_spanning_intron(*reverse_mate, forward_gene_end, reverse_gene_start, reverse_cigar_op, reverse_read_pos);
	const bool is_new = plan.count == 0;
	if (forward_has_intron && (!reverse_has_intron || forward_read_pos < reverse_mate->l_seq - reverse_read_pos)) {
		if (is_new) {
			plan_push(plan, forward_index, *forward_mate, false, forward_cigar_op + 1, CLIP_START);
			plan_push(plan, forward_index, *forward_mate, true, forward_cigar_op - 1, CLIP_END);
			if (reverse_mate != nullptr) {
				if (reverse_has_intron) plan_push(plan, reverse_index, *reverse_mate, false, reverse_cigar_op + 1, CLIP_START);
				else plan_push(plan, reverse_index, *reverse_mate, false, 0, CLIP_NONE);
			}
			return true;
		}
	} else if (reverse_has_intron) {
		if (is_new) {
			plan_push(plan, reverse_index, *reverse_mate, true, reverse_cigar_op + 1, CLIP_START);
			plan_push(plan, reverse_index, *reverse_mate, false, reverse_cigar_op - 1, CLIP_END);
			if (forward_mate != nullptr) {
				if (forward_has_intron) plan_push(plan, forward_index, *forward_mate, false, forward_cigar_op - 1, CLIP_END);
				else plan_push(plan, forward_index, *forward_mate, false, 0, CLIP_NONE);
			}
			return true;
		}
	} else if (forward_mate != nullptr && reverse_mate != nullptr && reverse_mate->pos >= reverse_gene_start && forward_mate->endpos() <= forward_gene_end) {
		if (is_new) {
			plan_push(plan, forward_index, *forward_mate, false, 0, CLIP_NONE);
			plan_push(plan, reverse_index, *reverse_mate, false, 0, CLIP_NONE);
		}
		return true;
	}
	return false;
}


struct CoverageBuild {
	uint32_t n_contigs;
	const uint64_t* window_offset;
	uint32_t* windows;
	uint8_t* fragment_starts;
	uint8_t* fragment_ends;
};
AGPU_HD uint64_t coverage_difference_slots(uint64_t windows, uint32_t n_contigs) { return windows + n_contigs; }

AGPU_HD void coverage_add(uint32_t* slot, uint32_t value) {
#if defined(__HIP_DEVICE_COMPILE__)
	__hip_atomic_fetch_add(slot, value, __ATOMIC_RELAXED, __HIP_MEMORY_SCOPE_AGENT);
#else
	__atomic_fetch_add(slot, value, __ATOMIC_RELAXED);
#endif
}
struct CoverageRange {
	uint64_t base; int64_t lo, hi;
	AGPU_HD void flush(uint32_t* differences) { if (hi > lo) { coverage_add(&differences[base + (uint64_t) lo], 1u); coverage_add(&differences[base + (uint64_t) hi], 0xFFFFFFFFu); } hi = lo = 0; }
	AGPU_HD void add(uint32_t* differences, uint64_t to_base, int64_t from, int64_t to) {
		if (hi > lo && to_base == base && from == hi) { hi = to; return; }
		flush(differences);
		base = to_base; lo = from; hi = to;
	}
};

AGPU_HD void add_fragment_to_coverage(const CoverageBuild& coverage, const Rec& mate1, uint16_t flag1, const Rec* mate2_or_null, bool is_chimeric) {
	const Rec& mate2 = (mate2_or_null == nullptr) ? mate1 : *mate2_or_null;
	if (coverage.windows == nullptr) return;
	if (mate1.contig < 0 || (uint32_t) mate1.contig >= coverage.n_contigs || mate2.contig < 0 || (uint32_t) mate2.contig >= coverage.n_contigs) return;
	const uint64_t begin1 = coverage.window_offset[mate1.contig], size1 = coverage.window_offset[mate1.contig + 1] - begin1;
	const uint64_t begin2 = coverage.window_offset[mate2.contig], size2 = coverage.window_offset[mate2.contig + 1] - begin2;
	if (size1 == 0 || size2 == 0) return;
	if ((flag1 & BAMF_PAIRED) && !(flag1 & BAMF_PROPER_PAIR)) is_chimeric = true;
	if (!is_chimeric) {
		if (!(flag1 & BAMF_REVERSE) || !(flag1 & BAMF_PAIRED)) { const uint64_t w = (uint64_t) (mate1.pos / COVERAGE_RESOLUTION); if (mate1.pos >= 0 && w < size1) coverage.fragment_starts[begin1 + w] = 1; }
		else { const uint64_t w = (uint64_t) (mate2.pos / COVERAGE_RESOLUTION); if (mate2.pos >= 0 && w < size2) coverage.fragment_starts[begin2 + w] = 1; }
	}
	int32_t position1 = mate1.pos, position2 = mate2.pos;
	int32_t position = position1 < position2 ? position1 : position2;
	int32_t window = position / COVERAGE_RESOLUTION;
	uint32_t i1 = 0, i2 = 0;
	const uint64_t slots1 = begin1 + (uint64_t) mate1.contig, slots2 = begin2 + (uint64_t) mate2.contig;
	CoverageRange pending; pending.base = 0; pending.lo = pending.hi = 0;
	while (true) {
		uint32_t op1 = 0, op2 = 0, length1, length2;
		if (i1 < mate1.n_cigar) { op1 = mate1.cigar(i1); length1 = op_consumes_reference(op1 & 15) ? op1 >> 4 : 0; }
		else { length1 = 0; if (position2 / COVERAGE_RESOLUTION > window) window = position2 / COVERAGE_RESOLUTION; }
		if (i2 < mate2.n_cigar) { op2 = mate2.cigar(i2); length2 = op_consumes_reference(op2 & 15) ? op2 >> 4 : 0; }
		else { length2 = 0; if (position1 / COVERAGE_RESOLUTION > window) window = position1 / COVERAGE_RESOLUTION; }
		uint32_t op;
		uint64_t begin, size;
		if (i1 < mate1.n_cigar && (position1 + (int32_t) length1 < position2 + (int32_t) length2 || i2 >= mate2.n_cigar)) {
			i1++;
			if (length1 == 0) continue;
			op = op1; begin = slots1; size = size1; position1 += (int32_t) length1; position = position1;
		} else if (i2 < mate2.n_cigar) {
			i2++;
			if (length2 == 0) continue;
			op = op2; begin = slots2; size = size2; position2 += (int32_t) length2; position = position2;
		} else {
			break;
		}
		if (op_consumes_query(op & 15)) {
			const int32_t last = position / COVERAGE_RESOLUTION;
			if (window <= last) {
				if (position >= 0) {
					const int64_t from = window > 0 ? window : 0;
					int64_t to = (position - last * COVERAGE_RESOLUTION >= COVERAGE_RESOLUTION / 2) ? (int64_t) last + 1 : (int64_t) last;
					if (to > (int64_t) size) to = (int64_t) size;
					if (to > from) pending.add(coverage.windows, begin, from, to);
				}
				window = last + 1;
			}
		} else {
			window = position / COVERAGE_RESOLUTION;
		}
	}
	pending.flush(coverage.windows);
	if (!is_chimeric) {
		if ((flag1 & BAMF_REVERSE) || !(flag1 & BAMF_PAIRED)) { const uint64_t w = (uint64_t) ((position1 - 1) / COVERAGE_RESOLUTION); if (position1 >= 1 && w < size1) coverage.fragment_ends[begin1 + w] = 1; }
		else { const uint64_t w = (uint64_t) ((position2 - 1) / COVERAGE_RESOLUTION); if (position2 >= 1 && w < size2) coverage.fragment_ends[begin2 + w] = 1; }
	}
}


struct IngestContext {
	IngestStream stream;
	AnnotationView annotation;
	GenomeView genome;
	CoverageBuild coverage;
	const uint8_t* record_bits;
	uint32_t max_itd_length;
	uint8_t external_duplicate_marking;
};

struct GroupTally { uint32_t malformed; uint32_t chimeric; uint32_t collision; };

template <class ViralCounter> AGPU_HD void replay_group(const IngestContext& ctx, const uint32_t* records, uint32_t n_records, FragmentPlan& plain, TandemPlan& itd, GroupTally& tally, ViralCounter& count_viral_read,
                                                        const Rec* names_of = nullptr, uint32_t length_of_names = 0 , int64_t hit_index_of_names = 0) {
	plan_clear(plain); plan_clear(itd.plan);
	itd.tandem.start = 0; itd.tandem.end = 0; itd.tandem.cigar[0] = itd.tandem.cigar[1] = itd.tandem.cigar[2] = 0; itd.tandem.record = NO_RECORD;
	itd.tandem.n_cigar = 0; itd.tandem.strand = 0; itd.tandem.first_in_pair = 0; itd.tandem.supplementary = 0;
	uint32_t parked = NO_RECORD;
	for (uint32_t k = 0; k < n_records; ++k) {
		const uint32_t index = records[k];
		const Rec record = load_record(ctx.stream, index);
		if (names_of != nullptr && k > 0 && !same_name(*names_of, length_of_names, hit_index_of_names, record, hit_index_of(ctx.stream, index, record))) tally.collision = 1;
		if (record.flag & BAMF_SUPPLEMENTARY) {
			if (is_clipped_at_correct_end(record)) plan_push(plain, index, record, true, 0, CLIP_NONE);
			else tally.malformed++;
			tally.chimeric = 1;
			continue;
		}
		uint32_t previous_index = NO_RECORD;
		Rec previous_storage;
		const Rec* previous = nullptr;
		bool is_read_through = false;
		uint16_t coverage_flag = record.flag;
		const bool discordant_mate = (record.flag & BAMF_PAIRED) && !(record.flag & BAMF_PROPER_PAIR);
		if (discordant_mate) {
			plan_push(plain, index, record, false, 0, CLIP_NONE);
			tally.chimeric = 1;
			coverage_flag = 0; is_read_through = true;
		} else {
			if (record.flag & BAMF_PAIRED) {
				if (parked == NO_RECORD) { parked = index; continue; }
				previous_index = parked; parked = NO_RECORD;
				previous_storage = load_record(ctx.stream, previous_index);
				previous = &previous_storage;
			}
			bool is_tandem_alignment = false;
			if (!clipped_sequence_is_adapter(record, previous) && (previous == nullptr || record.forward() != previous->forward())) {
				TandemAlignment tandem;
				bool found = false;
				AGPU_NOUNROLL for (uint32_t mate = 0; mate < 2 && !found; ++mate) found = is_tandem_duplication(mate ? previous : &record, mate ? previous_index : index, ctx.genome, ctx.max_itd_length, tandem);
				if (found) {
					plan_push(itd.plan, index, record, record.forward() == (bool) tandem.strand && !tandem.supplementary, 0, CLIP_NONE);
					if (previous != nullptr) plan_push(itd.plan, previous_index, *previous, previous->forward() == (bool) tandem.strand && !tandem.supplementary, 0, CLIP_NONE);
					if (itd.plan.count < 3) itd.tandem = tandem;
					plan_push_tandem(itd.plan);
					is_tandem_alignment = true;
				}
			}
			const bool record_has_sa = ctx.record_bits[index] & RECORD_HAS_SA, previous_has_sa = previous != nullptr && (ctx.record_bits[previous_index] & RECORD_HAS_SA);
			if ((record_has_sa && is_clipped_at_correct_end(record)) || (previous_has_sa && is_clipped_at_correct_end(*previous))) {
				plan_push(plain, index, record, false, 0, CLIP_NONE);
				if (previous != nullptr) plan_push(plain, previous_index, *previous, false, 0, CLIP_NONE);
				tally.chimeric = 1;
			} else if (!is_tandem_alignment) {
				is_read_through = extract_read_through_alignment(plain, index, record, previous_index, previous, ctx.annotation);
				if (record.contig >= 0 && (ctx.genome.contig_bits[record.contig] & CBIT_VIRAL)) {
					AGPU_NOUNROLL for (uint32_t mate = 0; mate < 2; ++mate) { const Rec* read = mate ? previous : &record; if (read != nullptr && is_pristine_alignment(*read)) count_viral_read((uint32_t) read->contig); }
				}
			}
		}
		if (!ctx.external_duplicate_marking || !(record.flag & BAMF_DUP)) add_fragment_to_coverage(ctx.coverage, record, coverage_flag, previous, is_read_through);
	}
}


struct Fragment3 { Aln a[3]; uint32_t n; bool single_end, duplicate; };

AGPU_HD bool disjoin_split_read_segments(Aln& split_read, Aln& supplementary) {
	const int min_remaining_supplementary_segment = 10;
	const unsigned int clipped_split_read = split_read.strand ? split_read.preclipping() : split_read.postclipping();
	const unsigned int clipped_supplementary = supplementary.strand ? supplementary.postclipping() : supplementary.preclipping();
	const int overlap = (int) split_read.sequence_length - clipped_split_read - clipped_supplementary;
	if (overlap <= 0) return true;
	const unsigned int clipped_op = supplementary.strand ? supplementary.n_cigar - 1 : 0;
	const unsigned int matching_op = supplementary.strand ? clipped_op - 1 : 1;
	if (supplementary.n_cigar < 2 || (supplementary.cigar(matching_op) & 15) != CIGAR_M || (int) (supplementary.cigar(matching_op) >> 4) < overlap + min_remaining_supplementary_segment) return false;
	const uint32_t clipped_element = supplementary.cigar(clipped_op), matching_element = supplementary.cigar(matching_op);
	supplementary.set_cigar(clipped_op, ((clipped_element >> 4) + overlap) << 4 | (clipped_element & 15));
	supplementary.set_cigar(matching_op, ((matching_element >> 4) - overlap) << 4 | (matching_element & 15));
	if (supplementary.strand) supplementary.end -= overlap; else supplementary.start += overlap;
	return true;
}

AGPU_HD void swap_alignments(Aln& x, Aln& y) { const Aln t = x; x = y; y = t; }
AGPU_HD void take_sequence(Aln& target, const Aln& source) { target.sequence_record = source.sequence_record; target.sequence_length = source.sequence_length; }

AGPU_HD bool normalize_plan(const IngestStream& in, const FragmentPlan& plan, const TandemAlignment* tandem, Fragment3& f) {
	f.single_end = plan.single_end; f.duplicate = plan.duplicate;
	const uint32_t size = plan.count;
	if (size < 2 || size > 3) return false;
	for (uint32_t k = 0; k < size; ++k) f.a[k] = materialize(in, plan.entry[k], tandem);
	for (uint32_t k = 0; k < size; ++k) if (f.a[k].n_cigar == 0) return false;
	Aln* a = f.a;
	f.n = size;
	if (plan.single_end) {
		if (!(size == 2 && (a[MATE1].supplementary != a[MATE2].supplementary))) return false;
		if (a[MATE1].end - a[MATE1].start > a[MATE2].end - a[MATE2].start) { a[2] = a[MATE2]; a[MATE2] = a[MATE1]; }
		else { a[2] = a[MATE1]; a[MATE1] = a[MATE2]; }
		f.n = 3;
		if (!a[MATE1].supplementary) take_sequence(a[SPLIT_READ], a[MATE1]);
		else if (!a[SPLIT_READ].supplementary) take_sequence(a[MATE1], a[SPLIT_READ]);
		else { take_sequence(a[MATE1], a[SUPPLEMENTARY]); take_sequence(a[SPLIT_READ], a[SUPPLEMENTARY]); }
		a[SUPPLEMENTARY].sequence_record = NO_RECORD; a[SUPPLEMENTARY].sequence_length = 0;
		if ((a[MATE1].cigar(0) & 15) == CIGAR_H) a[MATE1].set_cigar(0, a[MATE1].cigar(0) >> 4 << 4 | CIGAR_S);
		if ((a[MATE1].cigar(a[MATE1].n_cigar - 1) & 15) == CIGAR_H) a[MATE1].set_cigar(a[MATE1].n_cigar - 1, a[MATE1].cigar(a[MATE1].n_cigar - 1) >> 4 << 4 | CIGAR_S);
		if ((a[SPLIT_READ].cigar(0) & 15) == CIGAR_H) a[SPLIT_READ].set_cigar(0, a[SPLIT_READ].cigar(0) >> 4 << 4 | CIGAR_S);
		if ((a[SPLIT_READ].cigar(a[SPLIT_READ].n_cigar - 1) & 15) == CIGAR_H) {
			const uint32_t last = a[SPLIT_READ].n_cigar - 1;
			if (last >= a[MATE1].n_cigar) return false;
			a[SPLIT_READ].set_cigar(last, a[MATE1].cigar(last) >> 4 << 4 | CIGAR_S);
		}
		a[SUPPLEMENTARY].supplementary = true; a[MATE1].supplementary = false; a[SPLIT_READ].supplementary = false;
		bool flip_mate1_strand;
		const bool same = a[SPLIT_READ].strand == a[SUPPLEMENTARY].strand;
		const uint64_t length = (uint64_t) (uint32_t) a[SPLIT_READ].sequence_length;
		if (length - a[SPLIT_READ].preclipping() - (same ? a[SUPPLEMENTARY].postclipping() : a[SUPPLEMENTARY].preclipping()) <
		    length - a[SPLIT_READ].postclipping() - (same ? a[SUPPLEMENTARY].preclipping() : a[SUPPLEMENTARY].postclipping()))
			flip_mate1_strand = a[SPLIT_READ].strand == true;
		else
			flip_mate1_strand = a[SPLIT_READ].strand == false;
		a[MATE1].strand = complement_strand_if(a[MATE1].strand, flip_mate1_strand);
		a[SPLIT_READ].strand = complement_strand_if(a[SPLIT_READ].strand, !flip_mate1_strand);
		a[SUPPLEMENTARY].strand = complement_strand_if(a[SUPPLEMENTARY].strand, !flip_mate1_strand);
		a[MATE1].first_in_pair = !flip_mate1_strand;
		a[SPLIT_READ].first_in_pair = flip_mate1_strand;
		a[SUPPLEMENTARY].first_in_pair = flip_mate1_strand;
		if (!disjoin_split_read_segments(a[SPLIT_READ], a[SUPPLEMENTARY])) return false;
	} else {
		if (size == 3) {
			if (a[MATE1].supplementary) swap_alignments(a[MATE1], a[SUPPLEMENTARY]);
			else if (a[MATE2].supplementary) swap_alignments(a[MATE2], a[SUPPLEMENTARY]);
			if (a[SPLIT_READ].first_in_pair != a[SUPPLEMENTARY].first_in_pair) swap_alignments(a[MATE1], a[MATE2]);
			if (a[MATE1].supplementary || a[SPLIT_READ].supplementary || !a[SUPPLEMENTARY].supplementary) return false;
			if (a[MATE1].contig != a[SPLIT_READ].contig || a[MATE1].strand == a[SPLIT_READ].strand) return false;
			if (!disjoin_split_read_segments(a[SPLIT_READ], a[SUPPLEMENTARY])) return false;
		} else {
			if (a[MATE1].supplementary || a[MATE2].supplementary) return false;
		}
	}
	if ((a[MATE1].cigar(0) & 15) == CIGAR_H || (a[MATE1].cigar(a[MATE1].n_cigar - 1) & 15) == CIGAR_H ||
	    (a[MATE2].cigar(0) & 15) == CIGAR_H || (a[MATE2].cigar(a[MATE2].n_cigar - 1) & 15) == CIGAR_H)
		return false;
	return true;
}


AGPU_HD uint32_t decimal_digits(int64_t value, char* out ) {
	char reversed[21]; uint32_t n = 0;
	uint64_t magnitude = value < 0 ? (uint64_t) (-(value + 1)) + 1 : (uint64_t) value;
	do { reversed[n++] = (char) ('0' + magnitude % 10); magnitude /= 10; } while (magnitude > 0);
	uint32_t at = 0;
	if (value < 0) out[at++] = '-';
	while (n > 0) out[at++] = reversed[--n];
	return at;
}

struct FragmentName { const uint8_t* qname; uint32_t qname_length; char suffix[28]; uint32_t suffix_length; };
const uint32_t LENGTH_UNKNOWN = 0xFFFFFFFFu;
AGPU_HD FragmentName fragment_name(const Rec& representative, int64_t hit_index , bool itd, uint32_t length = LENGTH_UNKNOWN ) {
	FragmentName name;
	name.qname = representative.name; name.qname_length = length != LENGTH_UNKNOWN ? length : qname_length(representative);
	name.suffix[0] = ',';
	name.suffix_length = 1 + decimal_digits(hit_index, name.suffix + 1);
	if (itd) { name.suffix[name.suffix_length++] = 'I'; name.suffix[name.suffix_length++] = 'T'; name.suffix[name.suffix_length++] = 'D'; }
	return name;
}
AGPU_HD uint32_t name_length(const FragmentName& name) { return name.qname_length + name.suffix_length; }
AGPU_HD uint8_t name_byte(const FragmentName& name, uint32_t i) { return i < name.qname_length ? name.qname[i] : (i - name.qname_length < name.suffix_length ? (uint8_t) name.suffix[i - name.qname_length] : 0); }
AGPU_HD uint64_t name_chunk(const FragmentName& name, uint32_t chunk) {
	uint64_t value = 0;
	for (uint32_t k = 0; k < 8; ++k) value = value << 8 | name_byte(name, 8 * chunk + k);
	return value;
}
AGPU_HD int compare_names(const FragmentName& x, const FragmentName& y) {
	const uint32_t nx = name_length(x), ny = name_length(y), n = nx < ny ? nx : ny;
	const uint32_t qnames = x.qname_length < y.qname_length ? x.qname_length : y.qname_length, different = first_difference(x.qname, y.qname, qnames);
	if (different < qnames) return x.qname[different] < y.qname[different] ? -1 : 1;
	for (uint32_t i = qnames; i < n; ++i) { const uint8_t cx = name_byte(x, i), cy = name_byte(y, i); if (cx != cy) return cx < cy ? -1 : 1; }
	return nx < ny ? -1 : nx > ny ? 1 : 0;
}


struct FragmentSizes { uint32_t cigar_words, sequence_bytes, name_length; };
AGPU_HD uint32_t padded_sequence_bytes(uint32_t bases) { return (((bases + 1) / 2) + 3) & ~3u; }
AGPU_HD void fragment_sizes(const Fragment3& f, const Rec& representative, int64_t hit_index, bool itd, FragmentSizes& sizes, uint32_t length = LENGTH_UNKNOWN ) {
	uint32_t cigar_words = 0, sequence_bytes = 0;
	for (uint32_t s = 0; s < f.n; ++s) {
		cigar_words += f.a[s].n_cigar;
		if (s < 2) sequence_bytes += padded_sequence_bytes((uint32_t) f.a[s].sequence_length);
	}
	sizes.cigar_words = cigar_words; sizes.sequence_bytes = sequence_bytes;
	sizes.name_length = name_length(fragment_name(representative, hit_index, itd, length));
}

struct PackTarget {
	uint8_t* n_aln; uint8_t* fbits; uint32_t* group;
	uint16_t* contig[3]; int32_t* start[3]; int32_t* end[3]; uint8_t* abits[3]; uint32_t* cigar_offset[3]; uint16_t* cigar_count[3];
	uint32_t* cigar_pool; uint32_t* seq_offset[2]; uint32_t* seq_length[2]; uint8_t* seq_pool; char* names;
	uint64_t* name_offset;
	uint32_t* row_name_offset;
};

AGPU_HD uint32_t write_fragment(const IngestStream& in, const Fragment3& f, const FragmentName& name, uint64_t i, uint64_t cigar_at, uint64_t sequence_at, uint64_t name_at, uint32_t group, const PackTarget& out) {
	out.n_aln[i] = (uint8_t) f.n;
	out.fbits[i] = (f.single_end ? FBIT_SINGLE_END : 0) | (f.duplicate ? FBIT_DUPLICATE : 0);
	out.group[i] = group;
	uint32_t longest = 0;
	for (uint32_t s = 0; s < 3; ++s) {
		if (s >= f.n) {
			out.contig[s][i] = 0; out.start[s][i] = 0; out.end[s][i] = 0; out.abits[s][i] = 0; out.cigar_offset[s][i] = 0; out.cigar_count[s][i] = 0;
			if (s < 2) { out.seq_offset[s][i] = 0; out.seq_length[s][i] = 0; }
			continue;
		}
		const Aln& a = f.a[s];
		out.contig[s][i] = (uint16_t) a.contig; out.start[s][i] = a.start; out.end[s][i] = a.end;
		out.abits[s][i] = (a.strand ? ABIT_STRAND : 0) | (a.first_in_pair ? ABIT_FIRST_IN_PAIR : 0) | (a.supplementary ? ABIT_SUPPLEMENTARY : 0) | ABIT_PREDICTED_STRAND_AMBIGUOUS;
		out.cigar_offset[s][i] = (uint32_t) cigar_at; out.cigar_count[s][i] = (uint16_t) a.n_cigar;
		for (uint32_t k = 0; k < a.n_cigar; ++k) out.cigar_pool[cigar_at + k] = a.cigar(k);
		cigar_at += a.n_cigar;
		if (s < 2) {
			const uint32_t length = (uint32_t) a.sequence_length, bytes = (length + 1) / 2, padded = padded_sequence_bytes(length);
			out.seq_offset[s][i] = (uint32_t) (sequence_at / 4); out.seq_length[s][i] = length;
			if (length > longest) longest = length;
			if (length > 0) {
				const Rec source = load_record(in, a.sequence_record);
				uint32_t* target = (uint32_t*) (out.seq_pool + sequence_at);
				for (uint32_t w = 0; w < padded / 4; ++w) {
					uint32_t value = 0;
					if (4 * w + 4 < bytes) value = load_u32(source.seq_bytes + 4 * w);
					else for (uint32_t b = 0; b < 4; ++b) {
						const uint32_t at = 4 * w + b;
						if (at >= bytes) break;
						uint32_t byte = source.seq_bytes[at];
						if (at == bytes - 1 && (length & 1)) byte &= 0xF0u;
						value |= byte << (8 * b);
					}
					target[w] = value;
				}
			}
			sequence_at += padded;
		}
	}
	out.name_offset[i] = name_at;
	const uint32_t length = name_length(name);
	uint32_t copied = 0;
	for (; copied + 8 <= name.qname_length; copied += 8) { const uint64_t word = load_u64(name.qname + copied); __builtin_memcpy(out.names + name_at + copied, &word, 8); }
	for (uint32_t k = copied; k < name.qname_length; ++k) out.names[name_at + k] = (char) name.qname[k];
	for (uint32_t k = name.qname_length; k < length; ++k) out.names[name_at + k] = (char) name_byte(name, k);
	return longest;
}

AGPU_HD void row_sizes(const BatchView& b, const uint64_t* name_offset, uint64_t i, uint32_t& cigar_words, uint32_t& sequence_bytes, uint32_t& name_bytes) {
	cigar_words = 0; sequence_bytes = 0;
	for (uint32_t s = 0; s < b.n_aln[i]; ++s) {
		cigar_words += b.cigar_count[s][i];
		if (s < 2) sequence_bytes += padded_sequence_bytes(b.seq_length[s][i]);
	}
	name_bytes = name_offset ? (uint32_t) (name_offset[i + 1] - name_offset[i]) : 0;
}
AGPU_HD void copy_row(const BatchView& b, const uint8_t* pristine_fbits, const uint8_t* const* pristine_abits, const uint64_t* name_offset, const char* names, uint64_t i, uint64_t k,
                      uint64_t cigar_at, uint64_t sequence_at, uint64_t name_at, const PackTarget& out) {
	const uint32_t n_aln = b.n_aln[i];
	out.n_aln[k] = (uint8_t) n_aln; out.fbits[k] = pristine_fbits[i]; out.group[k] = b.group[i];
	for (uint32_t s = 0; s < 3; ++s) {
		out.contig[s][k] = b.contig[s][i]; out.start[s][k] = b.start[s][i]; out.end[s][k] = b.end[s][i]; out.abits[s][k] = pristine_abits[s][i];
		const uint32_t count = s < n_aln ? b.cigar_count[s][i] : 0;
		out.cigar_count[s][k] = (uint16_t) count; out.cigar_offset[s][k] = s < n_aln ? (uint32_t) cigar_at : 0;
		for (uint32_t c = 0; c < count; ++c) out.cigar_pool[cigar_at + c] = b.cigar_pool[b.cigar_offset[s][i] + c];
		cigar_at += count;
		if (s < 2) {
			const uint32_t length = s < n_aln ? b.seq_length[s][i] : 0, padded = padded_sequence_bytes(length);
			out.seq_length[s][k] = length; out.seq_offset[s][k] = s < n_aln ? (uint32_t) (sequence_at / 4) : 0;
			if (length > 0) {
				const uint32_t* source = (const uint32_t*) b.seq_pool + b.seq_offset[s][i];
				uint32_t* target = (uint32_t*) (out.seq_pool + sequence_at);
				for (uint32_t w = 0; w < padded / 4; ++w) target[w] = source[w];
			}
			sequence_at += padded;
		}
	}
	if (out.name_offset) out.name_offset[k] = name_at; else out.row_name_offset[k] = (uint32_t) name_at;
	if (name_offset) for (uint64_t c = name_offset[i]; c < name_offset[i + 1]; ++c) out.names[name_at + (c - name_offset[i])] = names[c];
}

AGPU_HD uint8_t strandedness_vote(const BatchView& b, const AnnotationView& ann, uint64_t i) {
	if (b.n_aln[i] != 3) return 0;
	const bool split_strand = b.abits[SPLIT_READ][i] & ABIT_STRAND, supplementary_strand = b.abits[SUPPLEMENTARY][i] & ABIT_STRAND;
	int32_t distance = b.start[SPLIT_READ][i] - b.start[SUPPLEMENTARY][i]; if (distance < 0) distance = -distance;
	if (!(b.contig[SPLIT_READ][i] == b.contig[SUPPLEMENTARY][i] && split_strand == supplementary_strand && distance < 400000)) return 0;
	AGPU_IDSET(genes);
	query_by_coordinate(ann.gene_index, b.contig[SPLIT_READ][i], b.start[SPLIT_READ][i], b.end[SPLIT_READ][i], IdentityMap(), genes);
	if (genes.n != 1 || genes.overflow) return 0;
	const uint32_t gene = genes.get(0);
	const int32_t position = split_strand ? b.start[SPLIT_READ][i] : b.end[SPLIT_READ][i];
	if (!is_breakpoint_spliced(ann, gene, split_strand, position)) return 0;
	const bool gene_strand = ann.gene_bits[gene] & GBIT_STRAND, mate1_strand = b.abits[MATE1][i] & ABIT_STRAND;
	const bool matching = ((b.abits[SPLIT_READ][i] & ABIT_FIRST_IN_PAIR) && split_strand == gene_strand) || ((b.abits[MATE1][i] & ABIT_FIRST_IN_PAIR) && mate1_strand == gene_strand);
	return matching ? 3 : 1;
}

}

#endif
```

Baseline: 61.68 million.

## Replace pointer-based fragment normalization with compact summaries and branchless selects

Fragment normalization and packing move from the full Fragment3/Aln representation to a compact FragmentSummary, with names built from a register-packed numeric suffix instead of a generic fragment name. Pointer-and-reference selections (previous mate, plan entries, tandem cigar) become value selects, so per-thread data stays in registers instead of scratch memory and divergence drops. The aim is lower register and scratch pressure and fewer divergent branches in the group-replay and pack kernels. In exchange, whole records are copied by value and both ITD and plain plans are always evaluated, which may add instructions.

```diff
diff --git a/arriba_amd/csrc/device/agpu_ingest.hip b/arriba_amd/csrc/device/agpu_ingest.hip
--- a/arriba_amd/csrc/device/agpu_ingest.hip
+++ b/arriba_amd/csrc/device/agpu_ingest.hip
@@ -280,7 +280,7 @@
 				qname_differs[g] = length != length_before || different < shorter;
 				bool unsorted;
 				if (different < shorter) unsorted = run_before.name[different] > representative.name[different];
-				else unsorted = compare_names(fragment_name(run_before, hit_index_of(ctx.stream, record_before, run_before), false, length_before), fragment_name(representative, hit, false, length)) >= 0;
+				else unsorted = compare_names(suffixed_name(run_before, hit_index_of(ctx.stream, record_before, run_before), false, length_before), suffixed_name(representative, hit, false, length)) >= 0;
 				if (unsorted) atomicOr(&counters[IC_RUNS_UNSORTED], 1u);
 			}
 		}
@@ -288,17 +288,19 @@
 		ViralCounter viral = { viral_counts };
 		replay_group(ctx, sorted_records + begin, n_records, plain_plan, itd_plan, tally, viral, RUNS ? &representative : nullptr, length, hit);
 		if (tally.collision) atomicOr(&counters[IC_COLLISION], 1u);
-		Fragment3 fragment;
+		FragmentSummary fragment;
 		AGPU_NOUNROLL for (uint32_t entry = 0; entry < 2; ++entry) {
-			const FragmentPlan& plan = entry ? itd_plan.plan : plain_plan;
+			FragmentPlan plan;
+			plan.count = either(entry, itd_plan.plan.count, plain_plan.count); plan.single_end = either(entry, itd_plan.plan.single_end, plain_plan.single_end); plan.duplicate = either(entry, itd_plan.plan.duplicate, plain_plan.duplicate); plan.reserved = 0;
+			plan.entry[0] = select_entry(entry, itd_plan.plan.entry[0], plain_plan.entry[0]); plan.entry[1] = select_entry(entry, itd_plan.plan.entry[1], plain_plan.entry[1]); plan.entry[2] = select_entry(entry, itd_plan.plan.entry[2], plain_plan.entry[2]);
 			bool ok = false;
 			if (plan.count > 0) {
-				ok = normalize_plan(ctx.stream, plan, entry ? &itd_plan.tandem : nullptr, fragment);
+				ok = normalize_summaries(ctx.stream, plan, itd_plan.tandem, fragment);
 				if (!ok) tally.malformed++;
 			}
 			valid[2 * (size_t) g + entry] = ok;
 			FragmentSizes mine; mine.cigar_words = 0; mine.sequence_bytes = 0; mine.name_length = 0;
-			if (ok) { if (entry) itd[g] = itd_plan; else plain[g] = plain_plan; fragment_sizes(fragment, representative, hit, entry, mine, length); }
+			if (ok) { if (entry) itd[g] = itd_plan; else plain[g] = plain_plan; summary_sizes(fragment, length, hit, entry, mine); }
 			sizes[2 * (size_t) g + entry] = mine;
 		}
 	}
@@ -376,11 +378,12 @@
 	if (i < n) {
 		const uint32_t ref = order[i], g = ref >> 1;
 		const bool is_itd = ref & 1;
-		Fragment3 f;
-		normalize_plan(in, is_itd ? itd[g].plan : plain[g], is_itd ? &itd[g].tandem : nullptr, f);
-		Rec storage;
-		const FragmentName name = name_of(in, group_first, ref, storage);
-		atomicMax(&block_max, write_fragment(in, f, name, i, cigar_base[i], sequence_base[i], name_base[i], group_id[i], out));
+		FragmentSummary f;
+		normalize_summaries(in, is_itd ? itd[g].plan : plain[g], itd[g].tandem, f);
+		const uint32_t first = group_first[g];
+		const Rec representative = load_record(in, first);
+		const SuffixedName name = suffixed_name(representative, hit_index_of(in, first, representative), is_itd, qname_length(representative));
+		atomicMax(&block_max, write_summary_fragment(in, f, name, i, cigar_base[i], sequence_base[i], name_base[i], group_id[i], out));
 	}
 	__syncthreads();
 	if (threadIdx.x == 0 && block_max) atomicMax(&counters[IC_MAX_READ_LENGTH], block_max);
diff --git a/arriba_amd/csrc/device/ingest_core.hpp b/arriba_amd/csrc/device/ingest_core.hpp
--- a/arriba_amd/csrc/device/ingest_core.hpp
+++ b/arriba_amd/csrc/device/ingest_core.hpp
@@ -67,6 +67,17 @@
 	AGPU_HD int32_t rlen(uint32_t n) const { int32_t l = 0; for (uint32_t i = 0; i < n; ++i) if (op_consumes_reference(op(i))) l += (int32_t) len(i); return l; }
 	AGPU_HD int32_t endpos() const { int32_t l = (!(flag & BAMF_UNMAP) && n_cigar > 0) ? rlen(n_cigar) : 1; return pos + (l == 0 ? 1 : l); }
 };
+
+template <class T> AGPU_HD T either(bool first, T a, T b) { return first ? a : b; }
+template <class T> AGPU_HD T one_of_three(uint32_t k, T a, T b, T c) { return k == 0 ? a : k == 1 ? b : c; }
+
+AGPU_HD Rec select_record(bool first, const Rec& a, const Rec& b) {
+	Rec r;
+	r.cigar_bytes = either(first, a.cigar_bytes, b.cigar_bytes); r.seq_bytes = either(first, a.seq_bytes, b.seq_bytes); r.name = either(first, a.name, b.name); r.aux = either(first, a.aux, b.aux); r.end = either(first, a.end, b.end);
+	r.contig = either(first, a.contig, b.contig); r.pos = either(first, a.pos, b.pos); r.l_seq = either(first, a.l_seq, b.l_seq);
+	r.n_cigar = either(first, a.n_cigar, b.n_cigar); r.l_read_name = either(first, a.l_read_name, b.l_read_name); r.flag = either(first, a.flag, b.flag);
+	return r;
+}
 
 AGPU_HD bool record_sizes_ok(const uint8_t* block, uint32_t block_size) {
 	if (block_size < 32) return false;
@@ -254,20 +265,23 @@
 };
 struct TandemPlan { FragmentPlan plan; TandemAlignment tandem; };
 
-AGPU_HD void plan_clear(FragmentPlan& plan) { plan.count = 0; plan.single_end = 0; plan.duplicate = 0; plan.reserved = 0; for (int k = 0; k < 3; ++k) { plan.entry[k].record = NO_RECORD; plan.entry[k].cigar_index = 0; plan.entry[k].clip = 0; plan.entry[k].supplementary = 0; } }
+AGPU_HD PlanEntry plan_entry(uint32_t record, uint32_t cigar_index, uint8_t clip, bool is_supplementary) { PlanEntry e; e.record = record; e.cigar_index = (uint16_t) cigar_index; e.clip = clip; e.supplementary = is_supplementary; return e; }
+AGPU_HD PlanEntry select_entry(bool first, const PlanEntry& a, const PlanEntry& b) { return plan_entry(either(first, a.record, b.record), either(first, a.cigar_index, b.cigar_index), either(first, a.clip, b.clip), either<bool>(first, a.supplementary, b.supplementary)); }
+AGPU_HD void plan_clear(FragmentPlan& plan) { plan.count = 0; plan.single_end = 0; plan.duplicate = 0; plan.reserved = 0; plan.entry[0] = plan.entry[1] = plan.entry[2] = plan_entry(NO_RECORD, 0, 0, false); }
+AGPU_HD void plan_set_if(PlanEntry& e, bool set, uint32_t record, uint32_t cigar_index, uint8_t clip, bool is_supplementary) {
+	e.record = either(set, record, e.record); e.cigar_index = either(set, (uint16_t) cigar_index, e.cigar_index); e.clip = either(set, clip, e.clip); e.supplementary = either<uint8_t>(set, is_supplementary, e.supplementary);
+}
+AGPU_HD void plan_append(FragmentPlan& plan, uint32_t record, uint32_t cigar_index, uint8_t clip, bool is_supplementary) {
+	const uint32_t at = plan.count;
+	plan_set_if(plan.entry[0], at == 0, record, cigar_index, clip, is_supplementary); plan_set_if(plan.entry[1], at == 1, record, cigar_index, clip, is_supplementary); plan_set_if(plan.entry[2], at == 2, record, cigar_index, clip, is_supplementary);
+	if (plan.count < 255) ++plan.count;
+}
 AGPU_HD void plan_push(FragmentPlan& plan, uint32_t record, const Rec& r, bool is_supplementary, uint32_t cigar_index, uint8_t clip) {
 	plan.single_end = !(r.flag & BAMF_PAIRED);
 	plan.duplicate = plan.duplicate || (r.flag & BAMF_DUP);
-	if (plan.count < 3) {
-		PlanEntry& e = plan.entry[plan.count];
-		e.record = record; e.cigar_index = (uint16_t) cigar_index; e.clip = clip; e.supplementary = is_supplementary;
-	}
-	if (plan.count < 255) ++plan.count;
-}
-AGPU_HD void plan_push_tandem(FragmentPlan& plan) {
-	if (plan.count < 3) { PlanEntry& e = plan.entry[plan.count]; e.record = NO_RECORD; e.cigar_index = 0; e.clip = PLAN_TANDEM; e.supplementary = 0; }
-	if (plan.count < 255) ++plan.count;
-}
+	plan_append(plan, record, cigar_index, clip, is_supplementary);
+}
+AGPU_HD void plan_push_tandem(FragmentPlan& plan) { plan_append(plan, NO_RECORD, 0, PLAN_TANDEM, false); }
 
 struct Aln {
 	const uint8_t* cigar_bytes;
@@ -372,11 +386,11 @@
 	return true;
 }
 
-AGPU_HD bool clipped_sequence_is_adapter(const Rec& mate1, const Rec* mate2) {
-	if (mate2 == nullptr) return false;
-	if (mate1.pos == mate2->pos && mate1.n_cigar > 0 && mate2->n_cigar > 0) {
-		if (!mate1.forward() && mate1.op(0) == CIGAR_S && mate2->forward() && mate2->op(mate2->n_cigar - 1) == CIGAR_S && mate1.len(0) == mate2->len(mate2->n_cigar - 1)) return true;
-		if (!mate2->forward() && mate2->op(0) == CIGAR_S && mate1.forward() && mate1.op(mate1.n_cigar - 1) == CIGAR_S && mate2->len(0) == mate1.len(mate1.n_cigar - 1)) return true;
+AGPU_HD bool clipped_sequence_is_adapter(const Rec& mate1, const Rec& mate2, bool has_mate2) {
+	if (!has_mate2) return false;
+	if (mate1.pos == mate2.pos && mate1.n_cigar > 0 && mate2.n_cigar > 0) {
+		if (!mate1.forward() && mate1.op(0) == CIGAR_S && mate2.forward() && mate2.op(mate2.n_cigar - 1) == CIGAR_S && mate1.len(0) == mate2.len(mate2.n_cigar - 1)) return true;
+		if (!mate2.forward() && mate2.op(0) == CIGAR_S && mate1.forward() && mate1.op(mate1.n_cigar - 1) == CIGAR_S && mate2.len(0) == mate1.len(mate1.n_cigar - 1)) return true;
 	}
 	return false;
 }
@@ -479,11 +493,11 @@
 			uint32_t clip_right = clipped_start ? r->l_seq - clipped_length : 0;
 			if (tandem_start > contig_pos) clip_left += tandem_start - contig_pos;
 			if (tandem_end < contig_pos + (int) clipped_length - 1) clip_right += contig_pos + clipped_length - 1 - tandem_end;
-			tandem.n_cigar = 0;
-			tandem.cigar[0] = tandem.cigar[1] = tandem.cigar[2] = 0;
-			if (clip_left > 0) tandem.cigar[tandem.n_cigar++] = clip_left << 4 | CIGAR_S;
-			tandem.cigar[tandem.n_cigar++] = (uint32_t) (tandem_end - tandem_start + 1) << 4 | CIGAR_M;
-			if (clip_right > 0) tandem.cigar[tandem.n_cigar++] = clip_right << 4 | CIGAR_S;
+			const uint32_t left = clip_left << 4 | CIGAR_S, match = (uint32_t) (tandem_end - tandem_start + 1) << 4 | CIGAR_M, right = clip_right << 4 | CIGAR_S;
+			tandem.cigar[0] = clip_left > 0 ? left : match;
+			tandem.cigar[1] = clip_left > 0 ? match : (clip_right > 0 ? right : 0);
+			tandem.cigar[2] = (clip_left > 0 && clip_right > 0) ? right : 0;
+			tandem.n_cigar = (uint8_t) (1 + (clip_left > 0) + (clip_right > 0));
 			return true;
 		}
 	}
@@ -527,15 +541,16 @@
 	}
 }
 
-AGPU_HD bool extract_read_through_alignment(FragmentPlan& plan, uint32_t record_index, const Rec& record, uint32_t previous_index, const Rec* previous, const AnnotationView& ann) {
-	const Rec* forward_mate = &record; const Rec* reverse_mate = previous;
-	uint32_t forward_index = record_index, reverse_index = previous_index;
-	if (!forward_mate->forward()) { const Rec* t = forward_mate; forward_mate = reverse_mate; reverse_mate = t; const uint32_t ti = forward_index; forward_index = reverse_index; reverse_index = ti; }
+AGPU_HD bool extract_read_through_alignment(FragmentPlan& plan, uint32_t record_index, const Rec& record, uint32_t previous_index, const Rec& previous, bool has_previous, const AnnotationView& ann) {
+	const bool swapped = !record.forward();
+	const Rec forward_mate = select_record(swapped, previous, record), reverse_mate = select_record(swapped, record, previous);
+	const bool has_forward = swapped ? has_previous : true, has_reverse = swapped ? true : has_previous;
+	const uint32_t forward_index = swapped ? previous_index : record_index, reverse_index = swapped ? record_index : previous_index;
 	ListRef forward_genes, reverse_genes;
-	if (forward_mate != nullptr) forward_genes = genes_at(ann.gene_index, forward_mate->contig, forward_mate->pos);
-	else forward_genes = genes_at(ann.gene_index, reverse_mate->contig, reverse_mate->pos);
-	if (reverse_mate != nullptr) reverse_genes = genes_at(ann.gene_index, reverse_mate->contig, reverse_mate->endpos());
-	else reverse_genes = genes_at(ann.gene_index, forward_mate->contig, forward_mate->endpos());
+	if (has_forward) forward_genes = genes_at(ann.gene_index, forward_mate.contig, forward_mate.pos);
+	else forward_genes = genes_at(ann.gene_index, reverse_mate.contig, reverse_mate.pos);
+	if (has_reverse) reverse_genes = genes_at(ann.gene_index, reverse_mate.contig, reverse_mate.endpos());
+	else reverse_genes = genes_at(ann.gene_index, forward_mate.contig, forward_mate.endpos());
 	const bool common_empty = !lists_intersect(forward_genes, reverse_genes);
 	if (!(common_empty && !(forward_genes.n == 0 && reverse_genes.n == 0))) return false;
 
@@ -547,33 +562,33 @@
 
 	uint32_t forward_cigar_op = 0, reverse_cigar_op = 0;
 	int32_t forward_read_pos = 0, reverse_read_pos = 0;
-	const bool forward_has_intron = (forward_mate == nullptr) ? false : find_spanning_intron(*forward_mate, forward_gene_end, reverse_gene_start, forward_cigar_op, forward_read_pos);
-	const bool reverse_has_intron = (reverse_mate == nullptr) ? false : find_spanning_intron(*reverse_mate, forward_gene_end, reverse_gene_start, reverse_cigar_op, reverse_read_pos);
+	const bool forward_has_intron = !has_forward ? false : find_spanning_intron(forward_mate, forward_gene_end, reverse_gene_start, forward_cigar_op, forward_read_pos);
+	const bool reverse_has_intron = !has_reverse ? false : find_spanning_intron(reverse_mate, forward_gene_end, reverse_gene_start, reverse_cigar_op, reverse_read_pos);
 	const bool is_new = plan.count == 0;
-	if (forward_has_intron && (!reverse_has_intron || forward_read_pos < reverse_mate->l_seq - reverse_read_pos)) {
+	if (forward_has_intron && (!reverse_has_intron || forward_read_pos < reverse_mate.l_seq - reverse_read_pos)) {
 		if (is_new) {
-			plan_push(plan, forward_index, *forward_mate, false, forward_cigar_op + 1, CLIP_START);
-			plan_push(plan, forward_index, *forward_mate, true, forward_cigar_op - 1, CLIP_END);
-			if (reverse_mate != nullptr) {
-				if (reverse_has_intron) plan_push(plan, reverse_index, *reverse_mate, false, reverse_cigar_op + 1, CLIP_START);
-				else plan_push(plan, reverse_index, *reverse_mate, false, 0, CLIP_NONE);
+			plan_push(plan, forward_index, forward_mate, false, forward_cigar_op + 1, CLIP_START);
+			plan_push(plan, forward_index, forward_mate, true, forward_cigar_op - 1, CLIP_END);
+			if (has_reverse) {
+				if (reverse_has_intron) plan_push(plan, reverse_index, reverse_mate, false, reverse_cigar_op + 1, CLIP_START);
+				else plan_push(plan, reverse_index, reverse_mate, false, 0, CLIP_NONE);
 			}
 			return true;
 		}
 	} else if (reverse_has_intron) {
 		if (is_new) {
-			plan_push(plan, reverse_index, *reverse_mate, true, reverse_cigar_op + 1, CLIP_START);
-			plan_push(plan, reverse_index, *reverse_mate, false, reverse_cigar_op - 1, CLIP_END);
-			if (forward_mate != nullptr) {
-				if (forward_has_intron) plan_push(plan, forward_index, *forward_mate, false, forward_cigar_op - 1, CLIP_END);
-				else plan_push(plan, forward_index, *forward_mate, false, 0, CLIP_NONE);
+			plan_push(plan, reverse_index, reverse_mate, true, reverse_cigar_op + 1, CLIP_START);
+			plan_push(plan, reverse_index, reverse_mate, false, reverse_cigar_op - 1, CLIP_END);
+			if (has_forward) {
+				if (forward_has_intron) plan_push(plan, forward_index, forward_mate, false, forward_cigar_op - 1, CLIP_END);
+				else plan_push(plan, forward_index, forward_mate, false, 0, CLIP_NONE);
 			}
 			return true;
 		}
-	} else if (forward_mate != nullptr && reverse_mate != nullptr && reverse_mate->pos >= reverse_gene_start && forward_mate->endpos() <= forward_gene_end) {
+	} else if (has_forward && has_reverse && reverse_mate.pos >= reverse_gene_start && forward_mate.endpos() <= forward_gene_end) {
 		if (is_new) {
-			plan_push(plan, forward_index, *forward_mate, false, 0, CLIP_NONE);
-			plan_push(plan, reverse_index, *reverse_mate, false, 0, CLIP_NONE);
+			plan_push(plan, forward_index, forward_mate, false, 0, CLIP_NONE);
+			plan_push(plan, reverse_index, reverse_mate, false, 0, CLIP_NONE);
 		}
 		return true;
 	}
@@ -607,8 +622,7 @@
 	}
 };
 
-AGPU_HD void add_fragment_to_coverage(const CoverageBuild& coverage, const Rec& mate1, uint16_t flag1, const Rec* mate2_or_null, bool is_chimeric) {
-	const Rec& mate2 = (mate2_or_null == nullptr) ? mate1 : *mate2_or_null;
+AGPU_HD void add_pair_to_coverage(const CoverageBuild& coverage, const Rec& mate1, uint16_t flag1, const Rec& mate2, bool is_chimeric) {
 	if (coverage.windows == nullptr) return;
 	if (mate1.contig < 0 || (uint32_t) mate1.contig >= coverage.n_contigs || mate2.contig < 0 || (uint32_t) mate2.contig >= coverage.n_contigs) return;
 	const uint64_t begin1 = coverage.window_offset[mate1.contig], size1 = coverage.window_offset[mate1.contig + 1] - begin1;
@@ -665,6 +679,7 @@
 		else { const uint64_t w = (uint64_t) ((position2 - 1) / COVERAGE_RESOLUTION); if (position2 >= 1 && w < size2) coverage.fragment_ends[begin2 + w] = 1; }
 	}
 }
+AGPU_HD void add_fragment_to_coverage(const CoverageBuild& coverage, const Rec& mate1, uint16_t flag1, const Rec* mate2_or_null, bool is_chimeric) { add_pair_to_coverage(coverage, mate1, flag1, mate2_or_null == nullptr ? mate1 : *mate2_or_null, is_chimeric); }
 
 
 struct IngestContext {
@@ -696,8 +711,8 @@
 			continue;
 		}
 		uint32_t previous_index = NO_RECORD;
-		Rec previous_storage;
-		const Rec* previous = nullptr;
+		Rec previous = record;
+		bool has_previous = false;
 		bool is_read_through = false;
 		uint16_t coverage_flag = record.flag;
 		const bool discordant_mate = (record.flag & BAMF_PAIRED) && !(record.flag & BAMF_PROPER_PAIR);
@@ -709,35 +724,35 @@
 			if (record.flag & BAMF_PAIRED) {
 				if (parked == NO_RECORD) { parked = index; continue; }
 				previous_index = parked; parked = NO_RECORD;
-				previous_storage = load_record(ctx.stream, previous_index);
-				previous = &previous_storage;
+				previous = load_record(ctx.stream, previous_index);
+				has_previous = true;
 			}
 			bool is_tandem_alignment = false;
-			if (!clipped_sequence_is_adapter(record, previous) && (previous == nullptr || record.forward() != previous->forward())) {
+			if (!clipped_sequence_is_adapter(record, previous, has_previous) && (!has_previous || record.forward() != previous.forward())) {
 				TandemAlignment tandem;
 				bool found = false;
-				AGPU_NOUNROLL for (uint32_t mate = 0; mate < 2 && !found; ++mate) found = is_tandem_duplication(mate ? previous : &record, mate ? previous_index : index, ctx.genome, ctx.max_itd_length, tandem);
+				AGPU_NOUNROLL for (uint32_t mate = 0; mate < (has_previous ? 2u : 1u) && !found; ++mate) { const Rec read = select_record(mate, previous, record); found = is_tandem_duplication(&read, mate ? previous_index : index, ctx.genome, ctx.max_itd_length, tandem); }
 				if (found) {
 					plan_push(itd.plan, index, record, record.forward() == (bool) tandem.strand && !tandem.supplementary, 0, CLIP_NONE);
-					if (previous != nullptr) plan_push(itd.plan, previous_index, *previous, previous->forward() == (bool) tandem.strand && !tandem.supplementary, 0, CLIP_NONE);
+					if (has_previous) plan_push(itd.plan, previous_index, previous, previous.forward() == (bool) tandem.strand && !tandem.supplementary, 0, CLIP_NONE);
 					if (itd.plan.count < 3) itd.tandem = tandem;
 					plan_push_tandem(itd.plan);
 					is_tandem_alignment = true;
 				}
 			}
-			const bool record_has_sa = ctx.record_bits[index] & RECORD_HAS_SA, previous_has_sa = previous != nullptr && (ctx.record_bits[previous_index] & RECORD_HAS_SA);
-			if ((record_has_sa && is_clipped_at_correct_end(record)) || (previous_has_sa && is_clipped_at_correct_end(*previous))) {
+			const bool record_has_sa = ctx.record_bits[index] & RECORD_HAS_SA, previous_has_sa = has_previous && (ctx.record_bits[previous_index] & RECORD_HAS_SA);
+			if ((record_has_sa && is_clipped_at_correct_end(record)) || (previous_has_sa && is_clipped_at_correct_end(previous))) {
 				plan_push(plain, index, record, false, 0, CLIP_NONE);
-				if (previous != nullptr) plan_push(plain, previous_index, *previous, false, 0, CLIP_NONE);
+				if (has_previous) plan_push(plain, previous_index, previous, false, 0, CLIP_NONE);
 				tally.chimeric = 1;
 			} else if (!is_tandem_alignment) {
-				is_read_through = extract_read_through_alignment(plain, index, record, previous_index, previous, ctx.annotation);
+				is_read_through = extract_read_through_alignment(plain, index, record, previous_index, previous, has_previous, ctx.annotation);
 				if (record.contig >= 0 && (ctx.genome.contig_bits[record.contig] & CBIT_VIRAL)) {
-					AGPU_NOUNROLL for (uint32_t mate = 0; mate < 2; ++mate) { const Rec* read = mate ? previous : &record; if (read != nullptr && is_pristine_alignment(*read)) count_viral_read((uint32_t) read->contig); }
+					AGPU_NOUNROLL for (uint32_t mate = 0; mate < (has_previous ? 2u : 1u); ++mate) { const Rec read = select_record(mate, previous, record); if (is_pristine_alignment(read)) count_viral_read((uint32_t) read.contig); }
 				}
 			}
 		}
-		if (!ctx.external_duplicate_marking || !(record.flag & BAMF_DUP)) add_fragment_to_coverage(ctx.coverage, record, coverage_flag, previous, is_read_through);
+		if (!ctx.external_duplicate_marking || !(record.flag & BAMF_DUP)) add_pair_to_coverage(ctx.coverage, record, coverage_flag, previous, is_read_through);
 	}
 }
 
@@ -928,6 +943,249 @@
 	return longest;
 }
 
+
+struct AlnSummary {
+	const uint8_t* cigar_bytes;
+	uint32_t record;
+	uint32_t n_cigar, shift;
+	uint32_t first, last, middle;
+	uint32_t patch_index, patch_value;
+	uint32_t sequence_record; int32_t sequence_length;
+	int32_t contig, start, end;
+	bool tandem, supplementary, first_in_pair, strand;
+	static AGPU_HD uint32_t element(const uint8_t* cigar_bytes, uint32_t n_cigar, uint32_t shift, uint32_t first, uint32_t last, uint32_t middle, uint32_t patch_index, uint32_t patch_value, bool tandem, uint32_t i) {
+		const bool held = i == 0 || i == n_cigar - 1 || i == patch_index || tandem;
+		uint32_t value = 0;
+		if (!held) value = load_u32(cigar_bytes + 4 * (size_t) (i + shift));
+		return i == 0 ? first : i == n_cigar - 1 ? last : i == patch_index ? patch_value : tandem ? middle : value;
+	}
+	AGPU_HD uint32_t cigar(uint32_t i) const { return element(cigar_bytes, n_cigar, shift, first, last, middle, patch_index, patch_value, tandem, i); }
+	AGPU_HD void set_cigar(uint32_t i, uint32_t value) {
+		const bool is_first = i == 0, is_last = !is_first && i == n_cigar - 1, is_inner = !is_first && !is_last;
+		first = either(is_first, value, first); last = either(is_last, value, last); patch_index = either(is_inner, i, patch_index); patch_value = either(is_inner, value, patch_value);
+	}
+	AGPU_HD uint32_t preclipping() const { const uint32_t op = first & 15; return (op == CIGAR_S || op == CIGAR_H) ? first >> 4 : 0; }
+	AGPU_HD uint32_t postclipping() const { const uint32_t c = either(n_cigar > 1, last, first), op = c & 15; return (op == CIGAR_S || op == CIGAR_H) ? c >> 4 : 0; }
+};
+
+AGPU_HD AlnSummary summarize(const IngestStream& in, const PlanEntry& e, const TandemAlignment& tandem) {
+	AlnSummary a;
+	a.shift = 0; a.middle = 0; a.patch_index = NO_RECORD; a.patch_value = 0; a.first = 0; a.last = 0;
+	a.tandem = e.clip == PLAN_TANDEM;
+	if (a.tandem) {
+		const Rec source = load_record(in, tandem.record);
+		a.cigar_bytes = source.cigar_bytes;
+		a.record = NO_RECORD;
+		a.supplementary = tandem.supplementary; a.first_in_pair = tandem.first_in_pair; a.strand = tandem.strand;
+		a.contig = source.contig; a.start = tandem.start; a.end = tandem.end;
+		a.n_cigar = tandem.n_cigar;
+		a.first = tandem.cigar[0]; a.middle = tandem.cigar[1]; a.last = either(tandem.n_cigar == 2, tandem.cigar[1], tandem.cigar[2]);
+		a.sequence_record = a.supplementary ? NO_RECORD : tandem.record;
+		a.sequence_length = a.supplementary ? 0 : source.l_seq;
+		return a;
+	}
+	const Rec r = load_record(in, e.record);
+	a.cigar_bytes = r.cigar_bytes;
+	a.record = e.record;
+	a.strand = r.forward(); a.first_in_pair = r.flag & BAMF_READ1; a.contig = r.contig; a.supplementary = e.supplementary;
+	a.sequence_record = e.supplementary ? NO_RECORD : e.record;
+	a.sequence_length = e.supplementary ? 0 : r.l_seq;
+	if (e.clip == CLIP_START) {
+		a.start = r.pos + r.rlen(e.cigar_index); a.end = r.endpos() - 1;
+		a.n_cigar = r.n_cigar - e.cigar_index + 1;
+		a.shift = (uint32_t) e.cigar_index - 1u;
+		a.first = (uint32_t) r.qlen(e.cigar_index) << 4 | (r.op(0) == CIGAR_H ? CIGAR_H : CIGAR_S);
+		if (a.n_cigar > 1) a.last = r.cigar(r.n_cigar - 1);
+	} else if (e.clip == CLIP_END) {
+		a.start = r.pos; a.end = r.pos + r.rlen((uint32_t) e.cigar_index + 1) - 1;
+		a.n_cigar = (uint32_t) e.cigar_index + 2;
+		a.first = r.cigar(0);
+		a.last = (uint32_t) (r.l_seq - r.qlen((uint32_t) e.cigar_index + 1)) << 4 | (r.op(r.n_cigar - 1) == CIGAR_H ? CIGAR_H : CIGAR_S);
+	} else {
+		a.start = r.pos; a.end = r.endpos() - 1;
+		a.n_cigar = r.n_cigar;
+		if (a.n_cigar > 0) a.first = r.cigar(0);
+		if (a.n_cigar > 1) a.last = r.cigar(r.n_cigar - 1);
+	}
+	return a;
+}
+
+AGPU_HD AlnSummary select_summary(uint32_t k, const AlnSummary& x, const AlnSummary& y, const AlnSummary& z) {
+	AlnSummary a;
+#define AGPU_PICK(member) a.member = one_of_three(k, x.member, y.member, z.member)
+	AGPU_PICK(cigar_bytes); AGPU_PICK(record); AGPU_PICK(n_cigar); AGPU_PICK(shift); AGPU_PICK(first); AGPU_PICK(last); AGPU_PICK(middle); AGPU_PICK(patch_index); AGPU_PICK(patch_value);
+	AGPU_PICK(sequence_record); AGPU_PICK(sequence_length); AGPU_PICK(contig); AGPU_PICK(start); AGPU_PICK(end); AGPU_PICK(tandem); AGPU_PICK(supplementary); AGPU_PICK(first_in_pair); AGPU_PICK(strand);
+#undef AGPU_PICK
+	return a;
+}
+
+struct FragmentSummary { AlnSummary mate1, mate2, supplementary; uint32_t n; bool single_end, duplicate; };
+
+AGPU_HD bool disjoin_split_read_summaries(const AlnSummary& split_read, AlnSummary& supplementary) {
+	const int min_remaining_supplementary_segment = 10;
+	const unsigned int clipped_split_read = split_read.strand ? split_read.preclipping() : split_read.postclipping();
+	const unsigned int clipped_supplementary = supplementary.strand ? supplementary.postclipping() : supplementary.preclipping();
+	const int overlap = (int) split_read.sequence_length - clipped_split_read - clipped_supplementary;
+	if (overlap <= 0) return true;
+	const unsigned int clipped_op = supplementary.strand ? supplementary.n_cigar - 1 : 0;
+	const unsigned int matching_op = supplementary.strand ? clipped_op - 1 : 1;
+	if (supplementary.n_cigar < 2) return false;
+	const uint32_t clipped_element = supplementary.cigar(clipped_op), matching_element = supplementary.cigar(matching_op);
+	if ((matching_element & 15) != CIGAR_M || (int) (matching_element >> 4) < overlap + min_remaining_supplementary_segment) return false;
+	supplementary.set_cigar(clipped_op, ((clipped_element >> 4) + overlap) << 4 | (clipped_element & 15));
+	supplementary.set_cigar(matching_op, ((matching_element >> 4) - overlap) << 4 | (matching_element & 15));
+	if (supplementary.strand) supplementary.end -= overlap; else supplementary.start += overlap;
+	return true;
+}
+
+AGPU_HD bool normalize_summaries(const IngestStream& in, const FragmentPlan& plan, const TandemAlignment& tandem, FragmentSummary& f) {
+	f.single_end = plan.single_end; f.duplicate = plan.duplicate;
+	const uint32_t size = plan.count;
+	f.n = size;
+	if (size < 2 || size > 3) return false;
+	const AlnSummary a0 = summarize(in, plan.entry[0], tandem), a1 = summarize(in, plan.entry[1], tandem);
+	const AlnSummary a2 = size == 3 ? summarize(in, plan.entry[2], tandem) : a1;
+	if (a0.n_cigar == 0 || a1.n_cigar == 0 || a2.n_cigar == 0) return false;
+	uint32_t slot1 = 0, slot2 = 1, slot3 = 2;
+	if (plan.single_end) {
+		if (!(size == 2 && (a0.supplementary != a1.supplementary))) return false;
+		if (a0.end - a0.start > a1.end - a1.start) { slot3 = 1; slot2 = 0; slot1 = 0; }
+		else { slot3 = 0; slot1 = 1; slot2 = 1; }
+		f.n = 3;
+	} else if (size == 3) {
+		if (a0.supplementary) { slot1 = 2; slot3 = 0; }
+		else if (a1.supplementary) { slot2 = 2; slot3 = 1; }
+		const bool split_read_first = either(slot2 == 1, a1.first_in_pair, a2.first_in_pair), supplementary_first = one_of_three(slot3, a0.first_in_pair, a1.first_in_pair, a2.first_in_pair);
+		if (split_read_first != supplementary_first) { const uint32_t t = slot1; slot1 = slot2; slot2 = t; }
+	}
+	f.mate1 = select_summary(slot1, a0, a1, a2); f.mate2 = select_summary(slot2, a0, a1, a2); f.supplementary = select_summary(slot3, a0, a1, a2);
+	AlnSummary& mate1 = f.mate1; AlnSummary& split_read = f.mate2; AlnSummary& supplementary = f.supplementary;
+	if (plan.single_end) {
+		if (mate1.supplementary) { mate1.sequence_record = supplementary.sequence_record; mate1.sequence_length = supplementary.sequence_length; split_read.sequence_record = supplementary.sequence_record; split_read.sequence_length = supplementary.sequence_length; }
+		supplementary.sequence_record = NO_RECORD; supplementary.sequence_length = 0;
+		if ((mate1.cigar(0) & 15) == CIGAR_H) mate1.set_cigar(0, mate1.cigar(0) >> 4 << 4 | CIGAR_S);
+		if ((mate1.cigar(mate1.n_cigar - 1) & 15) == CIGAR_H) mate1.set_cigar(mate1.n_cigar - 1, mate1.cigar(mate1.n_cigar - 1) >> 4 << 4 | CIGAR_S);
+		if ((split_read.cigar(0) & 15) == CIGAR_H) split_read.set_cigar(0, split_read.cigar(0) >> 4 << 4 | CIGAR_S);
+		if ((split_read.cigar(split_read.n_cigar - 1) & 15) == CIGAR_H) {
+			const uint32_t last = split_read.n_cigar - 1;
+			if (last >= mate1.n_cigar) return false;
+			split_read.set_cigar(last, mate1.cigar(last) >> 4 << 4 | CIGAR_S);
+		}
+		supplementary.supplementary = true; mate1.supplementary = false; split_read.supplementary = false;
+		bool flip_mate1_strand;
+		const bool same = split_read.strand == supplementary.strand;
+		const uint64_t length = (uint64_t) (uint32_t) split_read.sequence_length;
+		if (length - split_read.preclipping() - (same ? supplementary.postclipping() : supplementary.preclipping()) <
+		    length - split_read.postclipping() - (same ? supplementary.preclipping() : supplementary.postclipping()))
+			flip_mate1_strand = split_read.strand == true;
+		else
+			flip_mate1_strand = split_read.strand == false;
+		mate1.strand = complement_strand_if(mate1.strand, flip_mate1_strand);
+		split_read.strand = complement_strand_if(split_read.strand, !flip_mate1_strand);
+		supplementary.strand = complement_strand_if(supplementary.strand, !flip_mate1_strand);
+		mate1.first_in_pair = !flip_mate1_strand;
+		split_read.first_in_pair = flip_mate1_strand;
+		supplementary.first_in_pair = flip_mate1_strand;
+		if (!disjoin_split_read_summaries(split_read, supplementary)) return false;
+	} else {
+		if (size == 3) {
+			if (mate1.supplementary || split_read.supplementary || !supplementary.supplementary) return false;
+			if (mate1.contig != split_read.contig || mate1.strand == split_read.strand) return false;
+			if (!disjoin_split_read_summaries(split_read, supplementary)) return false;
+		} else {
+			if (mate1.supplementary || split_read.supplementary) return false;
+		}
+	}
+	if ((mate1.cigar(0) & 15) == CIGAR_H || (mate1.cigar(mate1.n_cigar - 1) & 15) == CIGAR_H ||
+	    (split_read.cigar(0) & 15) == CIGAR_H || (split_read.cigar(split_read.n_cigar - 1) & 15) == CIGAR_H)
+		return false;
+	return true;
+}
+
+struct NameSuffix {
+	uint64_t word0, word1, word2; uint32_t length;
+	AGPU_HD void prepend(uint8_t byte) { word2 = word2 << 8 | word1 >> 56; word1 = word1 << 8 | word0 >> 56; word0 = word0 << 8 | byte; ++length; }
+	AGPU_HD uint8_t byte(uint32_t j) const { return (uint8_t) (one_of_three(j >> 3, word0, word1, word2) >> (8 * (j & 7))); }
+};
+AGPU_HD NameSuffix name_suffix(int64_t hit_index, bool itd) {
+	NameSuffix s; s.word0 = itd ? 0x445449ull  : 0; s.word1 = 0; s.word2 = 0; s.length = itd ? 3 : 0;
+	uint64_t magnitude = hit_index < 0 ? (uint64_t) (-(hit_index + 1)) + 1 : (uint64_t) hit_index;
+	do { s.prepend((uint8_t) ('0' + magnitude % 10)); magnitude /= 10; } while (magnitude > 0);
+	if (hit_index < 0) s.prepend('-');
+	s.prepend(',');
+	return s;
+}
+struct SuffixedName { const uint8_t* qname; uint32_t qname_length; NameSuffix suffix; };
+AGPU_HD SuffixedName suffixed_name(const Rec& representative, int64_t hit_index, bool itd, uint32_t length ) { SuffixedName name; name.qname = representative.name; name.qname_length = length; name.suffix = name_suffix(hit_index, itd); return name; }
+AGPU_HD uint32_t name_length(const SuffixedName& name) { return name.qname_length + name.suffix.length; }
+AGPU_HD uint8_t name_byte(const SuffixedName& name, uint32_t i) { return i < name.qname_length ? name.qname[i] : (i - name.qname_length < name.suffix.length ? name.suffix.byte(i - name.qname_length) : 0); }
+AGPU_HD int compare_names(const SuffixedName& x, const SuffixedName& y) {
+	const uint32_t nx = name_length(x), ny = name_length(y), n = nx < ny ? nx : ny;
+	const uint32_t qnames = x.qname_length < y.qname_length ? x.qname_length : y.qname_length, different = first_difference(x.qname, y.qname, qnames);
+	if (different < qnames) return x.qname[different] < y.qname[different] ? -1 : 1;
+	for (uint32_t i = qnames; i < n; ++i) { const uint8_t cx = name_byte(x, i), cy = name_byte(y, i); if (cx != cy) return cx < cy ? -1 : 1; }
+	return nx < ny ? -1 : nx > ny ? 1 : 0;
+}
+
+AGPU_HD void summary_sizes(const FragmentSummary& f, uint32_t qname_length, int64_t hit_index, bool itd, FragmentSizes& sizes) {
+	sizes.cigar_words = f.mate1.n_cigar + f.mate2.n_cigar + (f.n == 3 ? f.supplementary.n_cigar : 0);
+	sizes.sequence_bytes = padded_sequence_bytes((uint32_t) f.mate1.sequence_length) + padded_sequence_bytes((uint32_t) f.mate2.sequence_length);
+	sizes.name_length = qname_length + name_suffix(hit_index, itd).length;
+}
+
+AGPU_HD uint32_t write_summary_slot(const IngestStream& in, const AlnSummary& a, bool present, uint32_t s, uint64_t i, uint64_t& cigar_at, uint64_t& sequence_at, const PackTarget& out) {
+	if (!present) {
+		out.contig[s][i] = 0; out.start[s][i] = 0; out.end[s][i] = 0; out.abits[s][i] = 0; out.cigar_offset[s][i] = 0; out.cigar_count[s][i] = 0;
+		if (s < 2) { out.seq_offset[s][i] = 0; out.seq_length[s][i] = 0; }
+		return 0;
+	}
+	out.contig[s][i] = (uint16_t) a.contig; out.start[s][i] = a.start; out.end[s][i] = a.end;
+	out.abits[s][i] = (a.strand ? ABIT_STRAND : 0) | (a.first_in_pair ? ABIT_FIRST_IN_PAIR : 0) | (a.supplementary ? ABIT_SUPPLEMENTARY : 0) | ABIT_PREDICTED_STRAND_AMBIGUOUS;
+	out.cigar_offset[s][i] = (uint32_t) cigar_at; out.cigar_count[s][i] = (uint16_t) a.n_cigar;
+	for (uint32_t k = 0; k < a.n_cigar; ++k) out.cigar_pool[cigar_at + k] = a.cigar(k);
+	cigar_at += a.n_cigar;
+	uint32_t length = 0;
+	if (s < 2) {
+		length = (uint32_t) a.sequence_length;
+		const uint32_t bytes = (length + 1) / 2, padded = padded_sequence_bytes(length);
+		out.seq_offset[s][i] = (uint32_t) (sequence_at / 4); out.seq_length[s][i] = length;
+		if (length > 0) {
+			const Rec source = load_record(in, a.sequence_record);
+			uint32_t* target = (uint32_t*) (out.seq_pool + sequence_at);
+			for (uint32_t w = 0; w < padded / 4; ++w) {
+				uint32_t value = 0;
+				if (4 * w + 4 < bytes) value = load_u32(source.seq_bytes + 4 * w);
+				else for (uint32_t b = 0; b < 4; ++b) {
+					const uint32_t at = 4 * w + b;
+					if (at >= bytes) break;
+					uint32_t byte = source.seq_bytes[at];
+					if (at == bytes - 1 && (length & 1)) byte &= 0xF0u;
+					value |= byte << (8 * b);
+				}
+				target[w] = value;
+			}
+		}
+		sequence_at += padded;
+	}
+	return length;
+}
+
+AGPU_HD uint32_t write_summary_fragment(const IngestStream& in, const FragmentSummary& f, const SuffixedName& name, uint64_t i, uint64_t cigar_at, uint64_t sequence_at, uint64_t name_at, uint32_t group, const PackTarget& out) {
+	out.n_aln[i] = (uint8_t) f.n;
+	out.fbits[i] = (f.single_end ? FBIT_SINGLE_END : 0) | (f.duplicate ? FBIT_DUPLICATE : 0);
+	out.group[i] = group;
+	const uint32_t length1 = write_summary_slot(in, f.mate1, true, 0, i, cigar_at, sequence_at, out);
+	const uint32_t length2 = write_summary_slot(in, f.mate2, true, 1, i, cigar_at, sequence_at, out);
+	write_summary_slot(in, f.supplementary, f.n == 3, 2, i, cigar_at, sequence_at, out);
+	out.name_offset[i] = name_at;
+	const uint32_t length = name_length(name);
+	uint32_t copied = 0;
+	for (; copied + 8 <= name.qname_length; copied += 8) { const uint64_t word = load_u64(name.qname + copied); __builtin_memcpy(out.names + name_at + copied, &word, 8); }
+	for (uint32_t k = copied; k < name.qname_length; ++k) out.names[name_at + k] = (char) name.qname[k];
+	for (uint32_t k = name.qname_length; k < length; ++k) out.names[name_at + k] = (char) name.suffix.byte(k - name.qname_length);
+	return length1 > length2 ? length1 : length2;
+}
+
 AGPU_HD void row_sizes(const BatchView& b, const uint64_t* name_offset, uint64_t i, uint32_t& cigar_words, uint32_t& sequence_bytes, uint32_t& name_bytes) {
 	cigar_words = 0; sequence_bytes = 0;
 	for (uint32_t s = 0; s < b.n_aln[i]; ++s) {
```

Result: slower. 58.07 million (-5.9%).
